# segments-ai/latent-diffusion-segmentation

Measured on AMD Instinct MI355X. Metric: denoising-steps/sec, higher is better.
Workload: dtype bf16; 1 GPU; 512x512 COCO-shaped latents (64x64x4), batch 8 per GPU, DDIM, self-conditioned 12-ch UNet without cross-attention (BASELINE configs[1]); batch_per_gpu=8, global_batch=8, latent=64, parallelism=dp1, ranks=1, backend=none, visible_devices=1

## Files before the change

### include/ldmseg_hip_ops.h

```cpp
#ifndef LDMSEG_HIP_OPS_H_
#define LDMSEG_HIP_OPS_H_
#include <stdint.h>
#ifdef __cplusplus
extern "C" {
#endif

int ldmseg_op_conv2d(const float* x, const float* x2, const float* w, const float* bias, int B, int Ci, int Ci2, int H,
                     int W, int Co, int k, int stride, int up, int dtype, float* out, void* stream);
int ldmseg_op_linear(const float* x, const float* w, const float* bias, const float* resid, const float* rowbias,
                     int rows_per_image, int M, int K, int N, int geglu, int silu, int splits, int dtype, float* out,
                     void* stream);
int ldmseg_op_chained_ff_out(const float* g, const float* h, const float* x, const float* w2, const float* b2, const float* wp,
                             const float* bp, int M, int C, int rows_per_image, int dtype, float* out, void* stream);
int ldmseg_op_groupnorm(const float* x, const float* x2, const float* gamma, const float* beta, int B, int C, int C2,
                        int HW, float eps, int silu, int dtype, float* out, void* stream);
int ldmseg_op_layernorm(const float* x, const float* gamma, const float* beta, int M, int C, float eps, int silu,
                        int dtype, float* out, void* stream);
int ldmseg_op_attention(const float* qkv, int B, int N, int C, int heads, int dtype, float* out, void* stream);
int ldmseg_op_attention_causal(const float* qkv, int B, int N, int C, int heads, int dtype, float* out, void* stream);
int ldmseg_op_attention_cross(const float* q, const float* kv, int B, int N, int S, int C, int heads, int dtype, float* out,
                              void* stream);
int ldmseg_op_attention_fp8(const float* qkv, int B, int N, int C, int heads, float* out, int time_iters, float* us_per_launch,
                            void* stream);
int ldmseg_op_convt2(const float* x, const float* w, const float* bias, int B, int Ci, int H, int W, int Co, int dtype,
                     float* out, void* stream);
int ldmseg_op_bilinear2x(const float* x, int B, int C, int H, int W, int dtype, float* out, void* stream);

int ldmseg_op_panoptic_from_decoder(const float* x4, int B, int C, int H4, int W4, int dtype, int in_h, int in_w,
                                    const int32_t* crop_boxes, const int32_t* out_sizes, const int64_t* out_offsets,
                                    int threshold_output, int threshold_mode, float mask_th, int count_th, double overlap_th,
                                    int64_t ignore_label, int32_t* labels, int32_t* panoptic, uint8_t* keep, int32_t* counts,
                                    int32_t* mask_counts, float* volume, void* stream);

int ldmseg_op_semseg_from_decoder(const float* x4, int B, int C, int H4, int W4, int dtype, int out_h, int out_w, float mask_th,
                                  int64_t ignore_label, const int64_t* targets, int64_t ignore_index, int num_classes,
                                  int64_t* preds, int64_t* counts, float* volume, void* stream);

int ldmseg_op_transformer_in(const float* x, const float* wp, const float* bp, const float* gamma, const float* beta, const float* wq,
                             const float* wk, const float* wv, int M, int C, float eps, int dtype, int mode, float* h_out, float* qkv_out,
                             int time_iters, float* us_per_call, void* stream);
int ldmseg_op_gn_transformer_in(const float* x, const float* gn_gamma, const float* gn_beta, float gn_eps, int images, int gn_mode,
                                const float* wp, const float* bp, const float* gamma, const float* beta, const float* wq,
                                const float* wk, const float* wv, int M, int C, float eps, int dtype, int mode, float* h_out,
                                float* qkv_out, int time_iters, float* us_per_call, void* stream);

int ldmseg_op_igemm(const float* x, const float* x2, const float* w, const float* bias, const float* resid,
                    const float* rowbias, int B, int Ci, int Ci2, int H, int W, int Co, int k, int stride, int up, int geglu,
                    int silu, int splits, int dtype, float* out, void* stream);
int ldmseg_op_conv3x3_plus_1x1(const float* h, const float* w2, const float* b2, const float* xs, const float* xs2, const float* ws,
                               const float* bs, int B, int C, int Cs, int Cs2, int H, int W, int Co, int splits, int dtype, float* out,
                               int iters, float* us_per_launch, void* stream);
int ldmseg_op_conv_groupnorm(const float* x, const float* w, const float* bias, const float* rowbias, const float* gamma,
                             const float* beta, int B, int Ci, int H, int W, int Co, float eps, int silu, int splits, int dtype,
                             float* out, void* stream);
int ldmseg_op_ln_linear(const float* x, const float* gamma, const float* beta, const float* w, const float* bias, int M, int K,
                        int N, float eps, int geglu, int dtype, float* out, void* stream);
int ldmseg_op_ln_linear_silu(const float* x, const float* gamma, const float* beta, const float* w, const float* bias, int M,
                             int K, int N, float eps, int dtype, float* out, void* stream);
int ldmseg_op_clip_patch_rows(const float* img, int B, int H, int W, int S, int P, const float* mean, const float* std,
                              int resample, int dtype, float* out, void* stream);
int ldmseg_op_clip_text_tokens(const int64_t* ids, const float* tok, const float* pos, int R, int T, int C, int vocab, int dtype,
                               float* out, void* stream);
int ldmseg_op_clip_text_final_ln(const float* x, const float* gamma, const float* beta, int M, int C, float eps, int dtype,
                                 float* out, void* stream);
int ldmseg_op_transformer_ff(const float* h, const float* x, const float* gamma, const float* beta, const float* w1, const float* b1,
                             const float* w2, const float* b2, const float* wp, const float* bp, int M, int C, float eps, int dtype,
                             int mode, float* out, int time_iters, float* us_per_call, void* stream);
int ldmseg_op_conv_out_tail(const float* x, const float* w, const float* bias, int B, int H, int W, float* eps_out, int ddim, int last,
                            const float* coef4, int pred_type, int clip, float clip_range, float* latents, float* cond,
                            const float* rgb, const uint8_t* known, const float* z0, const float* noise, float sa, float sb,
                            float* xin_out, void* stream);
int ldmseg_bench_igemm(const float* x, const float* x2, const float* w, const float* bias, const float* resid,
                       const float* rowbias, int B, int Ci, int Ci2, int H, int W, int Co, int k, int stride, int up, int geglu,
                       int silu, int splits, int dtype, int iters, float* us_per_launch, void* stream);
int ldmseg_bench_groupnorm(const float* gamma, const float* beta, int B, int C, int C2, int HW, int silu, int dtype, int iters,
                           float* us_per_launch, void* stream);
int ldmseg_bench_attention(const float* qkv, int B, int N, int C, int heads, int dtype, int iters, float* us_per_launch,
                           void* stream);
int ldmseg_igemm_last_kernel(char* buf, int n);
int ldmseg_op_igemm_plan(const int* desc, int dtype, int cus, char* buf, int n);
int ldmseg_op_groupnorm_plan(int B, int C, int C2, int HW, int groups, int dtype, int cus, int region_ok, char* buf, int n);
int ldmseg_op_conv_groupnorm_plan(int B, int Co, int HW, int dtype, char* buf, int n);
int ldmseg_op_attention_plan(int kind, int B, int N, int S, int C, int heads, int dtype, char* buf, int n);
int ldmseg_igemm_log(int enable);
int ldmseg_igemm_log_read(char* buf, int n);

int ldmseg_op_fastdiv(const int* n, int count, int d, int* q, void* stream);

#ifdef __cplusplus
}
#endif
#endif
```

### latent-diffusion-segmentation_amd/csrc/engine.hip

```cpp
#include <hip/hip_runtime.h>

#include <algorithm>
#include <array>
#include <cmath>
#include <cstdio>
#include <cstring>
#include <string>
#include <unordered_map>
#include <vector>

#include "../../include/ldmseg_hip.h"
#include "attn_plan.h"
#include "kernels.h"

using namespace ldmseg;

namespace {

thread_local std::string g_err;
int g_plan_epoch = 0;
int g_gnfold_mode = 1;
int g_ffp_mode = 1;
int fail(int code, const std::string& msg) {
  g_err = msg;
// ... 2148 lines not shown
  float* e1 = sinus + (size_t)h->temb_cap * 320;
  float* emb = e1 + (size_t)h->temb_cap * kTimeDim;
  float* table = emb + (size_t)h->temb_cap * kTimeDim;
  HIP_TRY(hipMemcpyAsync(ts, timesteps, (size_t)n_steps * sizeof(int64_t), hipMemcpyHostToDevice, s));
  for (int i0 = 0; i0 < n_steps; i0 += 64) {
    const int r = n_steps - i0 < 64 ? n_steps - i0 : 64;
    TRY(launch_time_embed(ts + i0, r, 0, r, sinus + (size_t)i0 * 320, s));
    TRY(launch_small_linear(sinus + (size_t)i0 * 320, h->te1_w, h->te1_b, e1 + (size_t)i0 * kTimeDim, r, 320, kTimeDim, 0, 1, s));
    TRY(launch_small_linear(e1 + (size_t)i0 * kTimeDim, h->te2_w, h->te2_b, emb + (size_t)i0 * kTimeDim, r, kTimeDim, kTimeDim, 0, 0, s));
    TRY(launch_small_linear(emb + (size_t)i0 * kTimeDim, h->tproj_w, h->tproj_b, table + (size_t)i0 * h->temb_total, r, kTimeDim,
                            h->temb_total, 1, 0, s));
  }
  *rows = table;
  return 0;
}

static int loop_reserve(ldmseg_unet* h, size_t n) {
  if (h->loop_elems >= n) return 0;
  HIP_TRY(hipDeviceSynchronize());
  if (h->cond) (void)hipFree(h->cond);
  if (h->eps) (void)hipFree(h->eps);
  h->cond = h->eps = nullptr;
  h->loop_elems = 0;
  HIP_TRY(hipMalloc((void**)&h->cond, n * sizeof(float)));
  HIP_TRY(hipMalloc((void**)&h->eps, n * sizeof(float)));
  h->loop_elems = n;
  return 0;
}

int ldmseg_unet_set_attention_fp8(ldmseg_unet* h, int min_tokens) {
  g_err.clear();
  if (!h || min_tokens < 0) return fail(LDMSEG_E_ARG, "bad argument");
  if (min_tokens > 0 && h->dt != DT_BF16) return fail(LDMSEG_E_ARG, "the fp8 attention path belongs to the bf16 perf mode");
  h->attn_fp8_min_tokens = min_tokens;
  h->plan_valid = false;
  return 0;
}

int ldmseg_unet_reserve(ldmseg_unet* h, int B, int L) {
  g_err.clear();
  if (!h) return fail(LDMSEG_E_ARG, "null argument");
  if (B < 1 || L < 8 || L % 8 != 0) return fail(LDMSEG_E_SHAPE, "L must be a positive multiple of 8, B >= 1");
  DeviceGuard dg(h->cfg.device);
  const int ci = h->cfg.in_channels;
  const PlanKey key{B, L, h->ctx_S, h->ctx_dim};
  TRY(plan_workspace(*h, &key, [&](bool dry, size_t scratch_base) {
    return unet_forward_impl(h, nullptr, ci, nullptr, 0, nullptr, 0, nullptr, 1, 0, B, L, nullptr, nullptr, dry, scratch_base);
  }));
  TRY(loop_reserve(h, (size_t)B * 4 * L * L));
  TRY(temb_reserve(h, 64));
  TRY(igemm_warm());
  return 0;
}

static int gn_backoff_update(ldmseg_unet* h) {
  if (h->gn_sync) {
    if (!h->gn_diag_host) {
      HIP_TRY(hipHostMalloc((void**)&h->gn_diag_host, sizeof(unsigned long long)));
      *h->gn_diag_host = 0;
    }
    const unsigned long long cur = *(volatile unsigned long long*)h->gn_diag_host;
    if (cur >= h->gn_diag_seen + 256) h->gn_backoff_calls = 8;
    else if (h->gn_backoff_calls > 0) --h->gn_backoff_calls;
    h->gn_diag_seen = cur;
  }
  return 0;
}

int ldmseg_sample_loop(ldmseg_unet* h, const ldmseg_sample_cfg* cfg, float* latents, const float* rgb_latents, int B, int L,
                       float* all_latents, void* stream) {
  g_err.clear();
  if (!h || !cfg || !latents || !rgb_latents || !cfg->timesteps || !cfg->coef) return fail(LDMSEG_E_ARG, "null argument");
  if (h->cfg.cross_attention) return fail(LDMSEG_E_ARG, "cross-attention handle: sample with ldmseg_sample_loop_guided");
  if (cfg->n_steps < 1) return fail(LDMSEG_E_ARG, "n_steps must be >= 1");
  if (B < 1 || L < 8 || L % 8 != 0) return fail(LDMSEG_E_SHAPE, "L must be a positive multiple of 8, B >= 1");
  if (cfg->prediction_type < 0 || cfg->prediction_type > 2) return fail(LDMSEG_E_ARG, "unknown prediction_type");
  for (int i = 0; i < cfg->n_steps; ++i)
    if (cfg->timesteps[i] < 0) return fail(LDMSEG_E_ARG, "negative timestep");
  DeviceGuard dg(h->cfg.device);
  hipStream_t s = (hipStream_t)stream;
  const size_t n = (size_t)B * 4 * L * L;
  const bool selfc = cfg->self_condition != 0;
  if ((h->cfg.in_channels == 12) != selfc) return fail(LDMSEG_E_ARG, "self_condition needs the 12-channel conv_in (and vice versa)");
  TRY(loop_reserve(h, n));
  const bool inpaint = cfg->known_dev != nullptr;
  if (inpaint && (!cfg->z0_dev || !cfg->noise_dev || !cfg->paste_coef)) return fail(LDMSEG_E_ARG, "inpainting needs z0, noise and paste_coef");
  if (selfc) HIP_TRY(hipMemsetAsync(h->cond, 0, n * sizeof(float), s));
  const float* temb_rows = nullptr;
  TRY(loop_time_embeddings(h, cfg->timesteps, cfg->n_steps, s, &temb_rows));
  TRY(gn_backoff_update(h));
  struct Clear { ldmseg_unet* u; ~Clear() { u->temb_override = nullptr; u->tail_req = nullptr; u->tail_done = false; u->xin_ready = false; u->xin_ptr = nullptr; } } clear{h};
  for (int i = 0; i < cfg->n_steps; ++i) {
    h->temb_override = temb_rows + (size_t)i * h->temb_total;
    const float* c = cfg->coef + 4 * i;
    DdimCoef dc{c[0], c[1], c[2], c[3], cfg->prediction_type, cfg->clip_sample, cfg->clip_sample_range, 0};
    const bool last = (i == cfg->n_steps - 1);
    StepTail st;
    st.ddim = 1; st.last = last ? 1 : 0; st.c = dc; st.latents = latents; st.cond = selfc ? h->cond : nullptr; st.rgb = rgb_latents;
    if (inpaint) { st.known = cfg->known_dev; st.z0 = cfg->z0_dev; st.noise = cfg->noise_dev; st.sa = cfg->paste_coef[2 * i]; st.sb = cfg->paste_coef[2 * i + 1]; }
    h->tail_req = &st;
    h->tail_done = false;
    TRY(unet_forward_checked(h, latents, 4, rgb_latents, 4, selfc ? h->cond : nullptr, selfc ? 4 : 0, nullptr, 1,
                             cfg->timesteps[i], B, L, h->eps, s));
    h->tail_req = nullptr;
    if (!h->tail_done) {
      if (!last) {
        TRY(launch_ddim_step(h->eps, latents, latents, selfc ? h->cond : nullptr, n, dc, s));
      } else {
        TRY(launch_ddim_step(h->eps, latents, nullptr, latents, n, dc, s));
      }
      if (inpaint)
        TRY(launch_inpaint_paste(latents, cfg->z0_dev, cfg->noise_dev, cfg->known_dev, cfg->paste_coef[2 * i],
                                 cfg->paste_coef[2 * i + 1], B, 4, L * L, s));
    }
    if (all_latents)
      HIP_TRY(hipMemcpyAsync(all_latents + (size_t)i * n, latents, n * sizeof(float), hipMemcpyDeviceToDevice, s));
  }
  if (h->gn_sync && h->gn_diag_host)
    HIP_TRY(hipMemcpyAsync(h->gn_diag_host, gn_sync_diag_ptr(h->gn_sync), sizeof(unsigned long long), hipMemcpyDeviceToHost, s));
  return 0;
}

int ldmseg_sample_loop_guided(ldmseg_unet* h, const ldmseg_sample_cfg* cfg, float* latents, const float* rgb_latents, int B, int L,
                              const float* ctx, int S, int ctx_dim, int multiplier, float guidance_scale, float* all_latents,
                              void* stream) {
  g_err.clear();
  if (!h || !cfg || !latents || !rgb_latents || !cfg->timesteps || !cfg->coef) return fail(LDMSEG_E_ARG, "null argument");
  if (cfg->n_steps < 1) return fail(LDMSEG_E_ARG, "n_steps must be >= 1");
  if (B < 1 || L < 8 || L % 8 != 0) return fail(LDMSEG_E_SHAPE, "L must be a positive multiple of 8, B >= 1");
  if (cfg->prediction_type < 0 || cfg->prediction_type > 2) return fail(LDMSEG_E_ARG, "unknown prediction_type");
  if (multiplier != 1 && multiplier != 2) return fail(LDMSEG_E_ARG, "multiplier must be 1 or 2");
  for (int i = 0; i < cfg->n_steps; ++i)
    if (cfg->timesteps[i] < 0) return fail(LDMSEG_E_ARG, "negative timestep");
  const bool selfc = cfg->self_condition != 0;
  if (selfc && multiplier == 2) return fail(LDMSEG_E_ARG, "self_condition with classifier-free guidance (multiplier 2) is not defined");
  if ((h->cfg.in_channels == 12) != selfc) return fail(LDMSEG_E_ARG, "self_condition needs the 12-channel conv_in (and vice versa)");
  if (cfg->known_dev || cfg->z0_dev || cfg->noise_dev || cfg->paste_coef) return fail(LDMSEG_E_ARG, "inpainting is not combined with guidance");
  TRY(set_ctx(h, ctx, S, ctx_dim));
  CtxClear cc{h};
  DeviceGuard dg(h->cfg.device);
  hipStream_t s = (hipStream_t)stream;
  const size_t n = (size_t)B * 4 * L * L;
  const int BB = multiplier * B;
  TRY(loop_reserve(h, (size_t)multiplier * n));
  float *lat2 = nullptr, *rgb2 = nullptr;
  if (multiplier == 2) {
    if (h->guide_elems < 4 * n) {
      HIP_TRY(hipDeviceSynchronize());
      if (h->guide_buf) (void)hipFree(h->guide_buf);
      h->guide_buf = nullptr; h->guide_elems = 0;
      HIP_TRY(hipMalloc((void**)&h->guide_buf, 4 * n * sizeof(float)));
      h->guide_elems = 4 * n;
    }
    lat2 = h->guide_buf;
    rgb2 = h->guide_buf + 2 * n;
    for (int k = 0; k < 2; ++k) {
      HIP_TRY(hipMemcpyAsync(lat2 + k * n, latents, n * sizeof(float), hipMemcpyDeviceToDevice, s));
      HIP_TRY(hipMemcpyAsync(rgb2 + k * n, rgb_latents, n * sizeof(float), hipMemcpyDeviceToDevice, s));
    }
  }
  if (selfc) HIP_TRY(hipMemsetAsync(h->cond, 0, n * sizeof(float), s));
  const float* temb_rows = nullptr;
  TRY(loop_time_embeddings(h, cfg->timesteps, cfg->n_steps, s, &temb_rows));
  TRY(gn_backoff_update(h));
  struct Clear { ldmseg_unet* u; ~Clear() { u->temb_override = nullptr; u->xin_ready = false; u->xin_ptr = nullptr; } } clear{h};
  for (int i = 0; i < cfg->n_steps; ++i) {
    h->temb_override = temb_rows + (size_t)i * h->temb_total;
    const float* c = cfg->coef + 4 * i;
    DdimCoef dc{c[0], c[1], c[2], c[3], cfg->prediction_type, cfg->clip_sample, cfg->clip_sample_range, 0};
    const bool last = (i == cfg->n_steps - 1);
    TRY(unet_forward_checked(h, multiplier == 2 ? lat2 : latents, 4, multiplier == 2 ? rgb2 : rgb_latents, 4,
                             selfc ? h->cond : nullptr, selfc ? 4 : 0, nullptr, 1, cfg->timesteps[i], BB, L, h->eps, s));
    h->ctx_kv_ready = true;
    TRY(launch_guided_step(h->eps, latents, selfc ? h->cond : nullptr, lat2, n, multiplier, guidance_scale, dc, last ? 1 : 0, s));
    if (all_latents)
      HIP_TRY(hipMemcpyAsync(all_latents + (size_t)i * n, latents, n * sizeof(float), hipMemcpyDeviceToDevice, s));
  }
  if (h->gn_sync && h->gn_diag_host)
    HIP_TRY(hipMemcpyAsync(h->gn_diag_host, gn_sync_diag_ptr(h->gn_sync), sizeof(unsigned long long), hipMemcpyDeviceToHost, s));
  return 0;
}

int ldmseg_unet_cf_fallbacks(ldmseg_unet* h, int64_t* count) {
  g_err.clear();
  if (!h || !count) return fail(LDMSEG_E_ARG, "null argument");
  DeviceGuard dg(h->cfg.device);
  unsigned long long n = 0;
  if (h->cf_sync) {
    HIP_TRY(hipDeviceSynchronize());
    HIP_TRY(hipMemcpy(&n, (const unsigned long long*)h->cf_sync + igemm_cf_bytes() / 8 - 1, sizeof n, hipMemcpyDeviceToHost));
  }
  *count = (int64_t)n;
  return 0;
}

int ldmseg_unet_gn_backoff(ldmseg_unet* h, int32_t* calls_left) {
  g_err.clear();
  if (!h || !calls_left) return fail(LDMSEG_E_ARG, "null argument");
  *calls_left = h->gn_backoff_calls;
  return 0;
}

int ldmseg_unet_gn_fallbacks(ldmseg_unet* h, int64_t* count) {
  g_err.clear();
  if (!h || !count) return fail(LDMSEG_E_ARG, "null argument");
  DeviceGuard dg(h->cfg.device);
  const long long n = h->gn_sync ? gn_coop_fallbacks(h->gn_sync) : 0;
  if (n < 0) return fail(LDMSEG_E_HIP, "reading the GroupNorm fallback counter failed");
  *count = n;
  return 0;
}

int ldmseg_bit_encode(const int64_t* ids, int B, int n_bits, int HW, int64_t ignore_label, float fill_value, float mul,
                      float add, float* bits, uint8_t* ignore_mask, void* stream) {
  g_err.clear();
  if (!ids || !bits || n_bits < 1 || n_bits > 31) return fail(LDMSEG_E_ARG, "bad bit_encode argument");
  TRY(launch_bit_encode(ids, bits, ignore_mask, B, n_bits, HW, ignore_label, fill_value, mul, add, (hipStream_t)stream));
  return 0;
}
int ldmseg_bit_decode(const float* x, int B, int n_bits, int HW, int64_t* ids, void* stream) {
  g_err.clear();
  if (!x || !ids || n_bits < 1 || n_bits > 24) return fail(LDMSEG_E_ARG, "bad bit_decode argument");
  TRY(launch_bit_decode(x, ids, B, n_bits, HW, (hipStream_t)stream));
  return 0;
}

int ldmseg_panoptic_postprocess(const float* logits, int B, int C, int H, int W, int threshold_output, int threshold_mode,
                                float mask_th, int count_th, double overlap_th, int64_t ignore_label, int32_t* labels,
                                int32_t* panoptic, uint8_t* keep, int32_t* counts, int32_t* mask_counts, void* stream) {
  g_err.clear();
  if (!logits || !labels || !panoptic || !keep || !counts || !mask_counts || B < 1 || C < 1 || C > 256 || H < 1 || W < 1 ||
      (threshold_mode != 0 && threshold_mode != 1))
    return fail(LDMSEG_E_ARG, "bad panoptic_postprocess argument");
  TRY(launch_panoptic_postprocess(logits, B, C, H * W, threshold_output, threshold_mode, mask_th, count_th, overlap_th,
                                  ignore_label, labels, panoptic, keep, counts, mask_counts, (hipStream_t)stream));
  return 0;
}

int ldmseg_profile_enable(int enable) {
  g_prof.on = enable != 0;
  return 0;
}
int ldmseg_profile_reset(void) {
  for (auto& f : g_prof.fam) {
    for (auto& e : f.ev) { g_prof.pool.push_back(e.first); g_prof.pool.push_back(e.second); }
    f.ev.clear();
    f.label.clear();
    f.lflops.clear();
    f.launches = 0;
    f.flops = f.bytes = 0;
  }
  return 0;
}
int ldmseg_profile_read(int family, int64_t* launches, double* total_ms, double* flops, double* bytes) {
  g_err.clear();
  if (family < 0 || family > 4) return fail(LDMSEG_E_ARG, "family must be 0..4");
  ProfFamily& f = g_prof.fam[family];
  double ms = 0;
  for (auto& e : f.ev) {
    HIP_TRY(hipEventSynchronize(e.second));
    float t = 0;
    HIP_TRY(hipEventElapsedTime(&t, e.first, e.second));
    ms += t;
  }
  if (launches) *launches = f.launches;
  if (total_ms) *total_ms = ms;
  if (flops) *flops = f.flops;
  if (bytes) *bytes = f.bytes;
  return 0;
}

int ldmseg_debug_set(int key, int value) {
  if (key == 2) { attention_set_qf1(value); return 0; }
  if (key == 1) { igemm_set_dbg(value); ++g_plan_epoch; return 0; }
  if (key == 5) { igemm_force_cfg(value); ++g_plan_epoch; return 0; }
  if (key == 8) { groupnorm_set_variant(value); ++g_plan_epoch; return 0; }
  if (key == 9) { igemm_set_cm_mode(value); ++g_plan_epoch; return 0; }
  if (key == 10) { groupnorm_set_coop(value, groupnorm_knob(11)); return 0; }
  if (key == 11) { groupnorm_set_coop(groupnorm_knob(10), value); return 0; }
  if (key == 12) { mlp_fused_set_mode(value); ++g_plan_epoch; return 0; }
  if (key == 13) { mlp_fused_set_dbg(value); return 0; }
  if (key == 14) { step_tail_set_mode(value); ++g_plan_epoch; return 0; }
  if (key == 16) { proj_qkv_set_mode(value); ++g_plan_epoch; return 0; }
  if (key == 15) { attention_mx_set_mode(value); ++g_plan_epoch; return 0; }
  if (key == 23) { igemm_set_cf_mode(value); ++g_plan_epoch; return 0; }
  if (key == 24) { igemm_set_table_override(value); ++g_plan_epoch; return 0; }
  if (key == 19) { igemm_set_xt_mode(value); ++g_plan_epoch; return 0; }
  if (key == 20) { g_ffp_mode = value ? 1 : 0; ++g_plan_epoch; return 0; }
  if (key == 22) { g_gnfold_mode = value < 0 ? 0 : value; ++g_plan_epoch; return 0; }
  if (key == 21) { igemm_set_up4_mode(value); ++g_plan_epoch; return 0; }
  if (key == 6 || key == 7) { ops_bench_knob(key, value); return 0; }
  static unsigned long long ts_ptr = 0;
  if (key == 3) { ts_ptr = (ts_ptr & 0xffffffff00000000ull) | (unsigned)value; igemm_set_tsbuf((void*)(uintptr_t)ts_ptr); return 0; }
  if (key == 4) { ts_ptr = (ts_ptr & 0xffffffffull) | ((unsigned long long)(unsigned)value << 32); igemm_set_tsbuf((void*)(uintptr_t)ts_ptr); return 0; }
  return fail(LDMSEG_E_ARG, "unknown debug key");
}

int ldmseg_debug_get(int key) {
  if (key == 1) return igemm_get_dbg();
  if (key == -1) return igemm_default_dbg();
  if (key == 8 || key == 11) return groupnorm_knob(key);
  if (key == 9) return igemm_get_cm_mode();
  if (key == 12) return mlp_fused_get_mode();
  if (key == 14) return step_tail_get_mode();
  if (key == 16) return proj_qkv_get_mode();
  if (key == 15) return attention_mx_get_mode();
  if (key == 23) return igemm_get_cf_mode();
  if (key == 19) return igemm_get_xt_mode();
  if (key == 20) return g_ffp_mode;
  if (key == 22) return g_gnfold_mode;
  if (key == 21) return igemm_get_up4_mode();
  if (key == 10) { const long long n = gn_coop_fallbacks(nullptr); return n > 0x7fffffffll ? 0x7fffffff : (int)n; }
  return 0;
}

int ldmseg_igemm_last_kernel(char* buf, int n) {
  if (!buf || n < 1) return LDMSEG_E_ARG;
  std::snprintf(buf, (size_t)n, "%s", igemm_dispatch_line(igemm_last_dispatch()).c_str());
  return 0;
}
int ldmseg_igemm_log(int enable) { igemm_log_enable(enable); return 0; }
int ldmseg_igemm_log_read(char* buf, int n) {
  if (!buf || n < 1) return LDMSEG_E_ARG;
  const std::string s = igemm_log_read();
  if ((int)s.size() + 1 > n) return LDMSEG_E_ARG;
  std::memcpy(buf, s.c_str(), s.size() + 1);
  return 0;
}

int ldmseg_profile_dump(const char* path) {
  g_err.clear();
  FILE* fp = std::fopen(path, "w");
  if (!fp) return fail(LDMSEG_E_ARG, "cannot open profile dump file");
  std::fprintf(fp, "family,label,ms,flops\n");
  for (int fi = 0; fi < 5; ++fi) {
    ProfFamily& f = g_prof.fam[fi];
    for (size_t i = 0; i < f.ev.size(); ++i) {
      (void)hipEventSynchronize(f.ev[i].second);
      float t = 0;
      (void)hipEventElapsedTime(&t, f.ev[i].first, f.ev[i].second);
      std::fprintf(fp, "%d,%s,%.6f,%.0f\n", fi, i < f.label.size() ? f.label[i].c_str() : "", t,
                   i < f.lflops.size() ? f.lflops[i] : 0.0);
    }
  }
  std::fclose(fp);
  return 0;
}

}
```

### latent-diffusion-segmentation_amd/csrc/kernels.h

```cpp
#pragma once
#include <hip/hip_runtime.h>
#include <stdint.h>

#include <string>
#include <vector>

#include "igemm_types.h"

namespace ldmseg {

struct FastDiv {
  unsigned mul = 0;
  int shift = 0;
  int d = 1;
};
inline FastDiv fastdiv_make(int d) {
  FastDiv f;
  f.d = d < 1 ? 1 : d;
  if (f.d == 1) return f;
  int s = 0;
  while ((1ll << s) < f.d) ++s;
  const unsigned long long num = 1ull << (31 + s);
  f.mul = (unsigned)((num + (unsigned long long)f.d - 1) / (unsigned long long)f.d);
  f.shift = s - 1;
  return f;
}

struct IgemmParams {
  const void* src0 = nullptr;
  const void* src1 = nullptr;
  int C0 = 0, C1 = 0;
  const void* src2 = nullptr;
  const void* src3 = nullptr;
  int C2 = 0, C3 = 0;
  int B = 0, Hi = 0, Wi = 0, Ho = 0, Wo = 0;
  int taps = 1;
  int pad = -1;
  int stride = 1;
  int up = 0;
  int up4 = 0;
  int cm = 0;
  int M = 0;
  int N = 0;
  int n_valid = 0;
  const void* W = nullptr;
  const float* bias = nullptr;
  const float* rowbias = nullptr;
  int rb_stride = 0;
  const float* rowstats = nullptr;
  const float* c1 = nullptr;
  const void* resid = nullptr;
  int ldr = 0;
  void* out = nullptr;
  int ldo = 0;
  int epi = EPI_STORE;
  int silu = 0;
  int cout = 0;
  int splits = 1;
  float* partial = nullptr;
  int no_finish = 0;
  unsigned long long* cf_ctr = nullptr;
  int cf = 0;
  unsigned cf_bytes = 0;
  int cf_poll_ticks = 20000;
  int cf_diag = 0;
  const void* zeros = nullptr;
  FastDiv fd_hwo, fd_wo, fd_nt, fd_ntiles, fd_nsplit, fd_tpt, fd_mphase;
  int x3 = 0;
  int w_dynamic = 0;
  int dbg = 0;
  unsigned long long* ts = nullptr;
};

int launch_igemm(const IgemmParams& p, int dtype, hipStream_t s);
size_t igemm_partial_bytes(const IgemmParams& p);
int igemm_warm();
int num_cus();
int igemm_plan_splits(const IgemmParams& p, int dtype);
size_t igemm_cf_bytes();
void igemm_set_cf_mode(int mode);
int igemm_get_cf_mode();
void igemm_set_table_override(int v);
void attention_set_qf1(int v);
void igemm_set_tsbuf(void* dev_buf);
void igemm_set_dbg(int flags);
void ops_bench_knob(int key, int value);
void igemm_set_cm_mode(int mode);
int igemm_get_cm_mode();
bool igemm_conv_cm(int hw, int ctot, int n, int k, int stride, int up, int dtype);
bool igemm_up4_ok(int B, int H, int W, int C, int N, int dtype);
void igemm_set_up4_mode(int on);
int igemm_get_up4_mode();
int launch_pack_up4(const float* w, void* out, int Co, int Ci, int Npad, int Cipad, int dtype, hipStream_t s);
bool igemm_xt_ok(const IgemmParams& p, int dtype);
void igemm_set_xt_mode(int on);
int igemm_get_xt_mode();
int launch_chain_weights(const float* wp, const float* w2, const float* b2, const float* bp, float* wcat, float* bcat, int C, hipStream_t s);
int launch_vec_add(const float* a, const float* b, float* out, int n, hipStream_t s);
int launch_split_planes(void* w, size_t nfloats, hipStream_t s);
int launch_concat_rows(const void* a, int K1, const void* b, int K2, void* out, int N, int dtype, hipStream_t s);
void igemm_force_cfg(int cfg);
int igemm_get_dbg();
int igemm_default_dbg();
IgemmDispatch igemm_last_dispatch();
int igemm_plan(const IgemmLaunchDesc& desc, int dtype, int cus, IgemmDispatch* d);
std::string igemm_dispatch_name(const IgemmDispatch& d);
std::string igemm_dispatch_line(const IgemmDispatch& d);
void igemm_log_enable(int level);
int igemm_log_level();
void igemm_log_note(const char* name);
std::string igemm_log_read();
std::string launch_name(const char* fmt, ...);
template <typename T>
constexpr const char* dtype_tag() { return sizeof(T) == 2 ? "bf16" : "f32"; }
#define LDMSEG_LAUNCH_AT(LEVEL, NAME, ...)                                                                  \
  do {                                                                                                      \
    if (::ldmseg::igemm_log_level() >= (LEVEL)) ::ldmseg::igemm_log_note(std::string(NAME).c_str());        \
    hipLaunchKernelGGL(__VA_ARGS__);                                                                        \
  } while (0)
#define LDMSEG_LAUNCH_GEMM(NAME, ...) LDMSEG_LAUNCH_AT(1, NAME, __VA_ARGS__)
#define LDMSEG_LAUNCH(NAME, ...) LDMSEG_LAUNCH_AT(2, NAME, __VA_ARGS__)
int igemm_pick_bn(int n_real, int epi);

struct GNParams {
  const void* src0 = nullptr; const void* src1 = nullptr;
  int C0 = 0, C1 = 0, B = 0, HW = 0, groups = 32;
  const float* gamma = nullptr; const float* beta = nullptr;
  float eps = 1e-5f; int silu = 0;
  void* out = nullptr;
  float* partial = nullptr;
  int nchunk = 0;
  int cpg = 0, vx = 0, ty = 0, per = 0;
  FastDiv fd_cpg, fd_vx, fd_aux;
  double inv_n = 0.0;
  void* sync_region = nullptr;
  unsigned long long* sync = nullptr;
  unsigned long long* sync_ctr = nullptr;
  unsigned long long* sync_diag = nullptr;
  int splits = 1;
  int coop_mode = 0;
  int poll_ticks = 10000;
  int poll_us = -1;
};
size_t gn_sync_bytes();
int gn_sync_init(void* region, hipStream_t s);
int gn_warm();
void groupnorm_set_coop(int mode, int poll_us);
long long gn_coop_fallbacks(const void* region);
const void* gn_sync_diag_ptr(const void* region);
int gn_nchunk(int B, int HW);
int launch_groupnorm(const GNParams& p, int dtype, hipStream_t s);
int launch_groupnorm_stats(const GNParams& p, int dtype, hipStream_t s);
bool finish_groupnorm_ok(int B, int HW, int C, int dtype);
int launch_finish_groupnorm(const IgemmParams& ip, const GNParams& g, int dtype, hipStream_t s);
void groupnorm_set_variant(int v);
int groupnorm_knob(int key);
struct GnDesc;
struct GnPlan;
int groupnorm_plan(const GnDesc& q, int cus, bool region_ok, GnPlan* pl);
int finish_groupnorm_plan(int B, int HW, int C, int dtype, GnPlan* pl);

int launch_layernorm(const void* x, void* y, const float* gamma, const float* beta, int M, int C,
                     float eps, int silu, int dtype, hipStream_t s);

int launch_attention(const void* qkv, void* out, int B, int N, int C, int heads, int dtype, hipStream_t s);
int launch_attention_causal(const void* qkv, void* out, int B, int N, int C, int heads, int dtype, hipStream_t s);
struct AttnKnobs;
struct AttnPlan;
AttnKnobs attention_knobs();
int launch_attn_v1_plan(const AttnPlan& p, const void* qkv, void* out, hipStream_t s);
int launch_attn3_plan(const AttnPlan& p, const void* qkv, void* out, hipStream_t s);
int launch_attn4_plan(const AttnPlan& p, const void* qkv, void* out, hipStream_t s);
int launch_attn_fp8_plan(const AttnPlan& p, const void* qkv, void* kv8, void* out, hipStream_t s);
int launch_attn_mx_plan(const AttnPlan& p, const void* qkv, void* kv8, void* out, hipStream_t s);
int launch_attn_cross_plan(const AttnPlan& p, const void* q, const void* kv, void* out, hipStream_t s);

int launch_attention_cross(const void* q, const void* kv, void* out, int B, int N, int S, int C, int heads, int dtype, hipStream_t s);
int launch_rows_to_dtype(const float* x, void* y, size_t n, int dtype, hipStream_t s);

bool mlp_fused_ok(int C, int dtype);
bool mlp_fused_proj();
void mlp_fused_set_mode(int m);
int mlp_fused_get_mode();
size_t mlp_fused_stream_bytes(int C);
int launch_pack_mlp_stream(const void* w1, const void* w2, const void* wp, void* out, int C, hipStream_t s);
bool proj_qkv_fused_ok(int C, int M, int dtype);
void proj_qkv_set_mode(int m);
int proj_qkv_get_mode();
size_t proj_qkv_stream_bytes(int C);
int launch_pack_proj_qkv_stream(const void* wp, const void* wqkv, void* out, int C, hipStream_t s);
struct GnFold {
  const float* partial = nullptr;
  const float* gamma = nullptr;
  const float* beta = nullptr;
  int nchunk = 0, HW = 0;
  float eps = 1e-6f;
};
bool proj_qkv_gn_fold_ok(int HW);
int proj_qkv_gn_chunks(int B, int HW);
int launch_proj_qkv_fused(const void* x, void* h, void* qkv, const void* stream, const float* bias4, const void* zeros, int M, int C, float eps,
                          const GnFold* gn, hipStream_t s);
int launch_mlp_fused(const void* h, void* out, const void* x2, const void* stream, const float* bias1, const float* bias2,
                     const float* bias3, const void* zeros, int M, int C, float eps, int proj, int rows_per_image, hipStream_t s);
void mlp_fused_set_dbg(int flags);
const void* igemm_zero_page();

int launch_rowstats(const void* x, float* stats, int M, int C, float eps, int dtype, hipStream_t s);
int launch_repack_rows_scaled(const float* w, void* out, const int* src_row_dev, int Npad, int K, const float* colscale,
                              int dtype, hipStream_t s);
int launch_rowsum(const void* W, const float* add, float* out, int N, int K, int dtype, hipStream_t s);

std::vector<int> geglu_row_map(int nout);
int launch_padded_bias(const float* src, int n, float* dst, int Npad, hipStream_t s);
struct LnFold {
  int parts = 1;
  const float* w[3] = {};
  const float* bias[3] = {};
  int Nper = 0, K = 0;
  int Npad = 0;
  const float* gamma = nullptr;
  const float* beta = nullptr;
  const std::vector<int>* row_map = nullptr;
  float scale = 0.f;
  int dtype = DT_BF16;
};
size_t ln_fold_scratch_bytes(const LnFold& f);
int launch_ln_fold(const LnFold& f, void* scratch, void* W, float* c1, float* bias, hipStream_t s);

int launch_clip_patch_rows(const float* img, void* rows, int B, int H, int W, int S, int P, int Kpad, const float* mean,
                           const float* std, int resample, int dtype, hipStream_t s);
int launch_clip_tokens(const void* patch, const float* cls, const float* pos, const float* gamma, const float* beta, void* h,
                       int B, int T, int C, float eps, int dtype, hipStream_t s);
int launch_clip_pooled_ln(const void* h, const float* gamma, const float* beta, float* out, int B, int T, int C, float eps,
                          int dtype, hipStream_t s);
int launch_clip_rows_to_f32(const void* x, float* y, size_t n, int dtype, hipStream_t s);

int launch_clip_text_tokens(const int64_t* ids, const float* tok, const float* pos, void* h, int R, int T, int C, int vocab,
                            int dtype, hipStream_t s);
int launch_clip_text_final_ln(const void* h, const float* gamma, const float* beta, float* out, int M, int C, float eps, int dtype,
                              hipStream_t s);

size_t attention_fp8_scratch_bytes(int B, int N, int C, int heads);
int launch_attention_fp8(const void* qkv, void* kv8_scratch, void* out, int B, int N, int C, int heads, hipStream_t s);
void attention_mx_set_mode(int m);
int attention_mx_get_mode();

int launch_pack_nchw(const float* x, void* y, int B, int C, int HW, int Cpad, float mul, float add,
                     int dtype, hipStream_t s);
int launch_pack_concat3(const float* a, int Ca, const float* b, int Cb, const float* c, int Cc,
                        void* y, int B, int HW, int Cpad, int dtype, hipStream_t s);

int launch_time_embed(const int64_t* t_dev, int t_count, int64_t t_host, int B, float* sinus ,
                      hipStream_t s);
int launch_small_linear(const float* x, const float* W, const float* bias, float* y, int B, int K, int N,
                        int silu_in, int silu_out, hipStream_t s);

int launch_bilinear2x_nchw(const void* x, float* y, int B, int H, int W, int C, int dtype, hipStream_t s);

int launch_bilinear2x_argmax(const void* x, int64_t* ids, float* prob, int B, int H, int W, int C, float mask_th,
                             int64_t ignore_label, int dtype, hipStream_t s);

int launch_repack_conv(const float* w, void* out, int Co, int Ci, int KH, int KW, int Npad, int Cipad,
                       int dtype, hipStream_t s, int cm_tile = 0);
int launch_repack_rows(const float* w, void* out, const int* src_row_dev, int Npad, int K, int dtype, hipStream_t s);
int launch_repack_convt2(const float* w, void* out, int Ci, int Co, int dtype, hipStream_t s);

struct DdimCoef { float sqrt_a_t, sqrt_b_t, sqrt_a_prev, sqrt_b_prev; int pred_type; int clip; float clip_range; int use_clipped; };
int launch_ddim_step(const float* eps, const float* x, float* prev, float* x0, size_t n, DdimCoef c, hipStream_t s);
int launch_guided_step(const float* eps, float* latents, float* cond, float* lat2, size_t n, int mult, float g, DdimCoef c,
                       int last, hipStream_t s);
struct StepTail {
  const void* x = nullptr;
  const void* w = nullptr;
  const float* bias = nullptr;
  const void* zeros = nullptr;
  int B = 0, H = 0, W = 0;
  float* eps_out = nullptr;
  int ddim = 0, last = 0;
  DdimCoef c{};
  float* latents = nullptr;
  float* cond = nullptr;
  const float* rgb = nullptr;
  void* xin_next = nullptr;
  const uint8_t* known = nullptr; const float* z0 = nullptr; const float* noise = nullptr;
  float sa = 0.f, sb = 0.f;
};
bool conv_out_tail_ok(int C, int H, int W, int dtype);
bool step_tail_fused();
void step_tail_set_mode(int m);
int step_tail_get_mode();
int launch_conv_out_tail(const StepTail& t, hipStream_t s);
int launch_inpaint_paste(float* cur, const float* z0, const float* noise, const uint8_t* known, float sa, float sb,
                         int B, int C, int HW, hipStream_t s);
int launch_add_noise(const float* x0, const float* noise, const int64_t* t_dev, const float* ac_dev, int n_train, float scale,
                     float* out, int B, size_t per, int remove, hipStream_t s);
int launch_softmax_rows(const float* s, void* p, int rows, int n, float scale, int dtype, hipStream_t st);
int launch_axpby(const float* x, float a, float b, float* y, size_t n, hipStream_t s);
int launch_panoptic_postprocess(const float* logits, int B, int C, int HW, int threshold_output, int threshold_mode,
                                float mask_th, int count_th, double overlap_th, int64_t ignore_label, int32_t* labels,
                                int32_t* panoptic, uint8_t* keep, int32_t* counts, int32_t* mask_counts, hipStream_t s);
int launch_panoptic_from_decoder(const void* x4, int B, int H4, int W4, int C, int dtype, int in_h, int in_w,
                                 const int32_t* boxes_host, const int32_t* sizes_host, const int64_t* offsets_host,
                                 int threshold_output, int threshold_mode, float mask_th, int count_th, double overlap_th,
                                 int64_t ignore_label, int32_t* labels, int32_t* panoptic, uint8_t* keep, int32_t* counts,
                                 int32_t* mask_counts, hipStream_t s, float* volume = nullptr,
                                 int mask_rule = 0);
int launch_semseg_meter(const int64_t* pred, const int64_t* gt, size_t n, int K, int64_t ignore_index, int64_t* counts, hipStream_t s);
int launch_semseg_from_decoder(const void* x4, int B, int H4, int W4, int C, int dtype, int oh, int ow, float mask_th,
                               int64_t ignore_label, const int64_t* targets, int64_t ignore_index, int K, int64_t* preds,
                               int64_t* counts, hipStream_t s, float* volume = nullptr);
int launch_pq_match(const int32_t* pred, const void* gt, int gt_format, int B, const int32_t* sizes_host, const int64_t* pred_offsets_host,
                    const int64_t* gt_offsets_host, const uint8_t* keep, int P, const int32_t* gt_counts_host, int Gpad,
                    const int32_t* slot_ids, const uint8_t* slot_crowd, const int64_t* slot_area, const int32_t* slot_meta,
                    int32_t* inter, int32_t* stats, double* match_iou, hipStream_t s);
int launch_bit_encode(const int64_t* ids, float* out, uint8_t* ignore, int B, int n, int HW, int64_t ignore_label,
                      float fill, float mul, float add, hipStream_t s);
int launch_bit_decode(const float* x, int64_t* out, int B, int n, int HW, hipStream_t s);
int launch_posterior_sample(const float* moments, const float* noise, float* out, int B, int HW, hipStream_t s);

}
```

### latent-diffusion-segmentation_amd/csrc/ops_api.hip

```cpp
#include <hip/hip_runtime.h>

#include <string>
#include <cstdio>
#include <cstdlib>
#include <cstring>
#include <vector>

#include "../../include/ldmseg_hip.h"
#include "common.h"
#include "attn_plan.h"
#include "gn_plan.h"
#include "kernels.h"

using namespace ldmseg;

static unsigned long long* op_cf_region() {
  static unsigned long long* r[64] = {};
  int dev = 0;
  if (hipGetDevice(&dev) != hipSuccess || dev < 0 || dev >= 64) return nullptr;
  if (!r[dev]) {
    void* q = nullptr;
    if (hipMalloc(&q, igemm_cf_bytes()) != hipSuccess) return nullptr;
    (void)hipMemset(q, 0, igemm_cf_bytes());
    r[dev] = (unsigned long long*)q;
// ... 373 lines not shown
  hipStream_t s = (hipStream_t)stream;
  if (M < 1 || C < 1) return -2;
  Temp t;
  void* xp = t.get((size_t)M * C * es(dtype));
  to_dev_dtype(x, xp, (size_t)M * C, dtype, s);
  return launch_clip_text_final_ln(xp, gamma, beta, out, M, C, eps, dtype, s);
}

int ldmseg_op_attention_cross(const float* q, const float* kv, int B, int N, int S, int C, int heads, int dtype, float* out,
                              void* stream) {
  hipStream_t s = (hipStream_t)stream;
  if (B < 1 || N < 1 || S < 1 || heads < 1 || C % heads) return -2;
  Temp t;
  void* qp = t.get((size_t)B * N * C * es(dtype));
  to_dev_dtype(q, qp, (size_t)B * N * C, dtype, s);
  void* kp = t.get((size_t)B * S * 2 * C * es(dtype));
  to_dev_dtype(kv, kp, (size_t)B * S * 2 * C, dtype, s);
  void* op = t.get((size_t)B * N * C * es(dtype));
  const int r = launch_attention_cross(qp, kp, op, B, N, S, C, heads, dtype, s);
  if (r) return r;
  from_dev_dtype(op, out, (size_t)B * N * C, dtype, s);
  return 0;
}

int ldmseg_op_convt2(const float* x, const float* w, const float* bias, int B, int Ci, int H, int W, int Co, int dtype,
                     float* out, void* stream) {
  hipStream_t s = (hipStream_t)stream;
  Temp t;
  if (Ci % bke(dtype) || Co % 4) return -2;
  void* xp = t.get((size_t)B * H * W * Ci * es(dtype));
  if (launch_pack_nchw(x, xp, B, Ci, H * W, Ci, 1.f, 0.f, dtype, s)) return -3;
  const int N = 4 * Co;
  const int bn = igemm_pick_bn(N, EPI_STORE);
  const int Np = rupi(N, bn);
  void* wp = t.get((size_t)Np * Ci * es(dtype));
  (void)hipMemsetAsync(wp, 0, (size_t)Np * Ci * es(dtype), s);
  if (launch_repack_convt2(w, wp, Ci, Co, dtype, s)) return -3;
  float* bp = (float*)t.get(Np * sizeof(float));
  (void)hipMemsetAsync(bp, 0, Np * sizeof(float), s);
  if (bias) for (int q = 0; q < 4; ++q) (void)hipMemcpyAsync(bp + q * Co, bias, Co * sizeof(float), hipMemcpyDeviceToDevice, s);
  void* op = t.get((size_t)B * 4 * H * W * Co * es(dtype));
  IgemmParams p;
  p.src0 = xp; p.C0 = Ci; p.B = B; p.Hi = p.Ho = H; p.Wi = p.Wo = W; p.M = B * H * W; p.N = Np; p.n_valid = N;
  p.W = wp; p.bias = bp; p.out = op; p.ldo = Co; p.epi = EPI_CONVT2; p.cout = Co;
  const int r = launch_igemm(p, dtype, s);
  if (r) return r;
  return unpack_nhwc(op, out, B, Co, 4 * H * W, Co, dtype, s);
}

int ldmseg_op_bilinear2x(const float* x, int B, int C, int H, int W, int dtype, float* out, void* stream) {
  hipStream_t s = (hipStream_t)stream;
  Temp t;
  void* xp = t.get((size_t)B * H * W * C * es(dtype));
  if (launch_pack_nchw(x, xp, B, C, H * W, C, 1.f, 0.f, dtype, s)) return -3;
  return launch_bilinear2x_nchw(xp, out, B, H, W, C, dtype, s);
}

static int g_bench_rot = 1, g_bench_ln = 0;
static int op_igemm_impl(const float* x, const float* x2, const float* w, const float* bias, const float* resid,
                         const float* rowbias, int B, int Ci, int Ci2, int H, int W, int Co, int k, int stride, int up, int geglu,
                         int silu, int splits, int dtype, float* out, void* stream, int time_iters, float* us_per_launch) {
  hipStream_t s = (hipStream_t)stream;
  Temp t;
  const int x3 = dtype == 2 ? 1 : (dtype == 3 ? 2 : 0);
  if (x3) dtype = DT_F32;
  const int a = bke(dtype);
  const int c0 = rupi(Ci, a), c1 = Ci2 ? rupi(Ci2, a) : 0;
  if (Ci2 && (Ci % a)) return -2;
  if (geglu && (k != 1 || Ci2 || (Co % 32))) return -2;
  void* xp = t.get((size_t)B * H * W * c0 * es(dtype));
  void* x2p = Ci2 ? t.get((size_t)B * H * W * c1 * es(dtype)) : nullptr;
  if (launch_pack_nchw(x, xp, B, Ci, H * W, c0, 1.f, 0.f, dtype, s)) return -3;
  if (Ci2 && launch_pack_nchw(x2, x2p, B, Ci2, H * W, c1, 1.f, 0.f, dtype, s)) return -3;
  const int epi = geglu ? EPI_GEGLU : EPI_STORE;
  const int bn = igemm_pick_bn(Co, epi);
  const int Np = rupi(Co, bn);
  const int ct = c0 + c1;
  const int cout = geglu ? Co / 2 : Co;
  const bool cm = !geglu && igemm_conv_cm(H * W, c0 + c1, Np, k, stride, up, dtype) && (Ci % a) == 0 && (!Ci2 || (Ci2 % a) == 0);
  void* wp = t.get((size_t)Np * k * k * ct * es(dtype));
  float* bp = padded_bias(t, geglu ? nullptr : bias, Co, Np, s);
  if (geglu) {
    std::vector<int> map = geglu_row_map(cout);
    map.resize(Np, -1);
    const int* dmap = upload_map(t, map, s);
    if (launch_repack_rows(w, wp, dmap, Np, ct, dtype, s)) return -3;
    if (bias && launch_repack_rows(bias, bp, dmap, Np, 1, DT_F32, s)) return -3;
  } else if (!Ci2) {
    if (launch_repack_conv(w, wp, Co, Ci, k, k, Np, c0, dtype, s, cm ? a : 0)) return -3;
  } else {
    void* w_cat = t.get((size_t)Co * ct * k * k * sizeof(float));
    (void)hipMemsetAsync(w_cat, 0, (size_t)Co * ct * k * k * sizeof(float), s);
    (void)hipMemcpy2DAsync(w_cat, (size_t)ct * k * k * sizeof(float), w, (size_t)(Ci + Ci2) * k * k * sizeof(float),
                           (size_t)(Ci + Ci2) * k * k * sizeof(float), Co, hipMemcpyDeviceToDevice, s);
    if (launch_repack_conv((const float*)w_cat, wp, Co, ct, k, k, Np, ct, dtype, s, cm ? a : 0)) return -3;
  }
  const int Hl = up ? 2 * H : H, Wl = up ? 2 * W : W;
  const int Ho = (k == 3 && stride == 2) ? (Hl - 1) / 2 + 1 : Hl, Wo = (k == 3 && stride == 2) ? (Wl - 1) / 2 + 1 : Wl;
  void* rp = nullptr;
  if (resid) {
    rp = t.get((size_t)B * Ho * Wo * cout * es(dtype));
    if (launch_pack_nchw(resid, rp, B, cout, Ho * Wo, cout, 1.f, 0.f, dtype, s)) return -3;
  }
  void* op = t.get((size_t)B * Ho * Wo * cout * es(dtype));
  IgemmParams p;
  p.src0 = xp; p.C0 = c0; p.src1 = x2p; p.C1 = c1;
  p.B = B; p.Hi = H; p.Wi = W; p.Ho = Ho; p.Wo = Wo; p.taps = k * k; p.stride = stride; p.up = up; p.cm = cm ? 1 : 0;
  p.M = B * Ho * Wo; p.N = Np; p.n_valid = cout; p.W = wp; p.bias = bp;
  p.rowbias = rowbias; p.rb_stride = Co;
  p.resid = rp; p.ldr = cout; p.out = op; p.ldo = cout; p.epi = epi; p.silu = silu;
  p.x3 = x3;
  if (x3 == 2 && launch_split_planes(wp, (size_t)Np * k * k * ct, s)) return -3;
  if (up && k == 3 && stride == 1 && !Ci2 && !geglu && !resid && !rowbias && !silu && igemm_up4_ok(B, H, W, c0, Np, dtype) && Ci == c0) {
    void* w4 = t.get((size_t)16 * Np * c0 * es(dtype));
    if (launch_pack_up4(w, w4, Co, Ci, Np, c0, dtype, s)) return -3;
    p.W = w4; p.taps = 4; p.up = 0; p.up4 = 1; p.Ho = H; p.Wo = W; p.M = 4 * B * H * W; p.cm = 0;
  }
  p.cf_ctr = op_cf_region();
  int sp = splits > 0 ? splits : igemm_plan_splits(p, dtype);
  if (sp > 1) { p.splits = sp; p.partial = (float*)t.get((size_t)sp * p.M * Np * sizeof(float)); }
  if (time_iters > 0 && g_bench_ln && sp <= 1 && !rowbias) {
    float* st = (float*)t.get((size_t)p.M * 2 * sizeof(float));
    float* c1z = (float*)t.get(Np * sizeof(float));
    (void)hipMemsetAsync(c1z, 0, Np * sizeof(float), s);
    std::vector<float> h((size_t)p.M * 2);
    for (int m = 0; m < p.M; ++m) { h[2 * m] = 0.f; h[2 * m + 1] = 1.f; }
    (void)hipMemcpy(st, h.data(), h.size() * sizeof(float), hipMemcpyHostToDevice);
    p.rowstats = st; p.c1 = c1z;
  }
  const int r = launch_igemm(p, dtype, s);
  if (r) return r;
  if (time_iters > 0 && us_per_launch) {
    const size_t wbytes = p.up4 ? (size_t)16 * Np * c0 * es(dtype) : (size_t)Np * k * k * ct * es(dtype);
    const void* wsrc = p.W;
    int rot = g_bench_rot < 1 ? 1 : g_bench_rot;
    std::vector<const void*> wc(1, wsrc);
    for (int i = 1; i < rot; ++i) {
      void* c = t.get(wbytes);
      if (!c) break;
      (void)hipMemcpyAsync(c, wsrc, wbytes, hipMemcpyDeviceToDevice, s);
      wc.push_back(c);
    }
    rot = (int)wc.size();
    *us_per_launch = time_launches(s, 3, time_iters, [&](int i) { p.W = wc[i % rot]; (void)launch_igemm(p, dtype, s); });
  }
  if (!out) return 0;
  return unpack_nhwc(op, out, B, cout, Ho * Wo, cout, dtype, s);
}

int ldmseg_op_conv3x3_plus_1x1(const float* h, const float* w2, const float* b2, const float* xs, const float* xs2, const float* ws,
                               const float* bs, int B, int C, int Cs, int Cs2, int H, int W, int Co, int splits, int dtype, float* out,
                               int iters, float* us_per_launch, void* stream) {
  hipStream_t s = (hipStream_t)stream;
  Temp t;
  if (dtype != DT_BF16 || C % 64 || Cs % 64 || Cs2 % 64 || !h || !w2 || !xs || !ws) return -2;
  const int HW = H * W, cs = Cs + Cs2;
  void* hp = t.get((size_t)B * HW * C * 2);
  void* xp = t.get((size_t)B * HW * Cs * 2);
  void* x2p = Cs2 ? t.get((size_t)B * HW * Cs2 * 2) : nullptr;
  if (launch_pack_nchw(h, hp, B, C, HW, C, 1.f, 0.f, dtype, s)) return -3;
  if (launch_pack_nchw(xs, xp, B, Cs, HW, Cs, 1.f, 0.f, dtype, s)) return -3;
  if (Cs2 && launch_pack_nchw(xs2, x2p, B, Cs2, HW, Cs2, 1.f, 0.f, dtype, s)) return -3;
  const int Np = rupi(Co, igemm_pick_bn(Co, EPI_STORE));
  void* w2p = t.get((size_t)Np * 9 * C * 2);
  void* wsp = t.get((size_t)Np * cs * 2);
  void* wx = t.get((size_t)Np * (9 * C + cs) * 2);
  if (launch_repack_conv(w2, w2p, Co, C, 3, 3, Np, C, dtype, s)) return -3;
  if (launch_repack_conv(ws, wsp, Co, cs, 1, 1, Np, cs, dtype, s)) return -3;
  if (launch_concat_rows(w2p, 9 * C, wsp, cs, wx, Np, dtype, s)) return -3;
  float* b2p = padded_bias(t, b2, Co, Np, s);
  float* bsp = padded_bias(t, bs, Co, Np, s);
  float* bx = (float*)t.get(Np * sizeof(float));
  if (launch_vec_add(b2p, bsp, bx, Np, s)) return -3;
  void* op = t.get((size_t)B * HW * Co * 2);
  IgemmParams p;
  p.src0 = hp; p.C0 = C; p.src2 = xp; p.C2 = Cs; p.src3 = x2p; p.C3 = Cs2;
  p.B = B; p.Hi = p.Ho = H; p.Wi = p.Wo = W; p.taps = 9; p.stride = 1;
  p.M = B * HW; p.N = Np; p.n_valid = Co; p.W = wx; p.bias = bx; p.out = op; p.ldo = Co; p.epi = EPI_STORE;
  if (!igemm_xt_ok(p, dtype)) return -4;
  p.cf_ctr = op_cf_region();
  const int sp = splits > 0 ? splits : igemm_plan_splits(p, dtype);
  if (sp > 1) { p.splits = sp; p.partial = (float*)t.get((size_t)sp * p.M * Np * sizeof(float)); }
  const int r = launch_igemm(p, dtype, s);
  if (r) return r;
  if (iters > 0 && us_per_launch) *us_per_launch = time_launches(s, 0, iters, [&](int) { (void)launch_igemm(p, dtype, s); });
  if (!out) return 0;
  return unpack_nhwc(op, out, B, Co, HW, Co, dtype, s);
}

int ldmseg_op_igemm_plan(const int* desc, int dtype, int cus, char* buf, int n) {
  if (!desc || !buf || n < 1 || cus < 1 || dtype < 0 || dtype > 3) return -2;
  IgemmLaunchDesc q;
  static_assert(sizeof q == 17 * sizeof(int), "ldmseg_op_igemm_plan takes the fields of IgemmLaunchDesc in order");
  std::memcpy(&q, desc, sizeof q);
  if (dtype >= 2) { q.x3 = dtype - 1; dtype = DT_F32; }
  IgemmDispatch d;
  if (const int r = igemm_plan(q, dtype, cus, &d)) return r;
  std::snprintf(buf, (size_t)n, "%s", igemm_dispatch_line(d).c_str());
  return 0;
}

int ldmseg_op_fastdiv(const int* n, int count, int d, int* q, void* stream) {
  if (!n || !q || count < 0 || d < 1) return -2;
  const FastDiv f = fastdiv_make(d);
  hipLaunchKernelGGL(fastdiv_probe_kernel, dim3((count + 255) / 256), dim3(256), 0, (hipStream_t)stream, n, count, f, q);
  return hipGetLastError() == hipSuccess ? 0 : -3;
}
}
namespace ldmseg {
void ops_bench_knob(int key, int value) {
  if (key == 6) g_bench_rot = value;
  if (key == 7) g_bench_ln = value;
}
}
extern "C" {
int ldmseg_op_igemm(const float* x, const float* x2, const float* w, const float* bias, const float* resid,
                    const float* rowbias, int B, int Ci, int Ci2, int H, int W, int Co, int k, int stride, int up, int geglu,
                    int silu, int splits, int dtype, float* out, void* stream) {
  return op_igemm_impl(x, x2, w, bias, resid, rowbias, B, Ci, Ci2, H, W, Co, k, stride, up, geglu, silu, splits, dtype, out,
                       stream, 0, nullptr);
}
int ldmseg_bench_igemm(const float* x, const float* x2, const float* w, const float* bias, const float* resid,
                       const float* rowbias, int B, int Ci, int Ci2, int H, int W, int Co, int k, int stride, int up, int geglu,
                       int silu, int splits, int dtype, int iters, float* us_per_launch, void* stream) {
  return op_igemm_impl(x, x2, w, bias, resid, rowbias, B, Ci, Ci2, H, W, Co, k, stride, up, geglu, silu, splits, dtype, nullptr,
                       stream, iters, us_per_launch);
}
int ldmseg_bench_attention(const float* qkv, int B, int N, int C, int heads, int dtype, int iters, float* us_per_launch,
                           void* stream) {
  hipStream_t s = (hipStream_t)stream;
  Temp t;
  void* qp = t.get((size_t)B * N * 3 * C * es(dtype));
  to_dev_dtype(qkv, qp, (size_t)B * N * 3 * C, dtype, s);
  void* op = t.get((size_t)B * N * C * es(dtype));
  int err = 0;
  *us_per_launch = time_launches(s, 3, iters, [&](int) { if (const int r = launch_attention(qp, op, B, N, C, heads, dtype, s)) err = err ? err : r; });
  return err;
}

}
namespace {
int op_ln_linear_impl(const float* x, const float* gamma, const float* beta, const float* w, const float* bias, int M, int K,
                      int N, float eps, int geglu, int silu, int dtype, float* out, void* stream) {
  hipStream_t s = (hipStream_t)stream;
  Temp t;
  const int x3 = dtype == 2 ? 1 : (dtype == 3 ? 2 : 0);
  if (x3) dtype = DT_F32;
  if (K % bke(dtype)) return -2;
  void* xp = t.get((size_t)M * K * es(dtype));
  to_dev_dtype(x, xp, (size_t)M * K, dtype, s);
  const int epi = geglu ? EPI_GEGLU : EPI_STORE;
  const int bn = (!geglu && N % 160 != 0) ? 160 : igemm_pick_bn(N, epi);
  const int Np = rupi(N, bn);
  const int nout = geglu ? N / 2 : N;
  std::vector<int> map;
  if (geglu) { map = geglu_row_map(nout); map.resize(Np, -1); }
  LnFold f;
  f.w[0] = w; f.bias[0] = bias; f.Nper = N; f.K = K; f.Npad = Np; f.gamma = gamma; f.beta = beta; f.dtype = dtype;
  if (geglu) f.row_map = &map;
  void* wp = t.get((size_t)Np * K * es(dtype));
  float* c1 = (float*)t.get(Np * sizeof(float));
  float* c2 = (float*)t.get(Np * sizeof(float));
  if (launch_ln_fold(f, t.get(ln_fold_scratch_bytes(f)), wp, c1, c2, s)) return -3;
  float* stats = (float*)t.get((size_t)M * 2 * sizeof(float));
  if (launch_rowstats(xp, stats, M, K, eps, dtype, s)) return -3;
  void* op = t.get((size_t)M * nout * es(dtype));
  IgemmParams p;
  p.src0 = xp; p.C0 = K; p.B = 1; p.Hi = p.Ho = M; p.Wi = p.Wo = 1;
  p.M = M; p.N = Np; p.n_valid = nout; p.W = wp; p.bias = c2; p.rowstats = stats; p.c1 = c1;
  p.out = op; p.ldo = nout; p.epi = epi; p.silu = silu;
  p.x3 = x3;
  if (x3 == 2 && launch_split_planes(wp, (size_t)Np * K, s)) return -3;
  const int sp = igemm_plan_splits(p, dtype);
  if (sp > 1) { p.splits = sp; p.partial = (float*)t.get((size_t)sp * M * Np * sizeof(float)); }
  const int r = launch_igemm(p, dtype, s);
  if (r) return r;
  from_dev_dtype(op, out, (size_t)M * nout, dtype, s);
  return 0;
}
}
extern "C" {
int ldmseg_op_ln_linear(const float* x, const float* gamma, const float* beta, const float* w, const float* bias, int M, int K,
                        int N, float eps, int geglu, int dtype, float* out, void* stream) {
  return op_ln_linear_impl(x, gamma, beta, w, bias, M, K, N, eps, geglu, 0, dtype, out, stream);
}
int ldmseg_op_ln_linear_silu(const float* x, const float* gamma, const float* beta, const float* w, const float* bias, int M,
                             int K, int N, float eps, int dtype, float* out, void* stream) {
  return op_ln_linear_impl(x, gamma, beta, w, bias, M, K, N, eps, 0, 1, dtype, out, stream);
}
int ldmseg_op_clip_patch_rows(const float* img, int B, int H, int W, int S, int P, const float* mean, const float* std,
                              int resample, int dtype, float* out, void* stream) {
  hipStream_t s = (hipStream_t)stream;
  if (B < 1 || P < 1 || S < P || S % P) return -2;
  Temp t;
  const int Kpad = rupi(3 * P * P, 64), G = S / P;
  const size_t n = (size_t)B * G * G * Kpad;
  void* rows = t.get(n * es(dtype));
  const int r = launch_clip_patch_rows(img, rows, B, H, W, S, P, Kpad, mean, std, resample, dtype, s);
  if (r) return r;
  from_dev_dtype(rows, out, n, dtype, s);
  return 0;
}

int ldmseg_op_transformer_ff(const float* h, const float* x, const float* gamma, const float* beta, const float* w1, const float* b1,
                             const float* w2, const float* b2, const float* wp, const float* bp, int M, int C, float eps, int dtype,
                             int mode, float* out, int time_iters, float* us_per_call, void* stream) {
  hipStream_t s = (hipStream_t)stream;
  Temp t;
  const int rows_per_image = (M % 4096 == 0) ? 4096 : 0;
  if (C % bke(dtype) || (mode != 0 && (dtype != DT_BF16 || !mlp_fused_stream_bytes(C)))) return -2;
  const int N1 = 8 * C;
  void* hp = t.get((size_t)M * C * es(dtype));
  void* h0 = t.get((size_t)M * C * es(dtype));
  void* xp = t.get((size_t)M * C * es(dtype));
  void* op = t.get((size_t)M * C * es(dtype));
  to_dev_dtype(h, h0, (size_t)M * C, dtype, s);
  to_dev_dtype(x, xp, (size_t)M * C, dtype, s);
  const std::vector<int> map = geglu_row_map(4 * C);
  LnFold f;
  f.w[0] = w1; f.bias[0] = b1; f.Nper = N1; f.K = C; f.Npad = N1; f.gamma = gamma; f.beta = beta; f.row_map = &map; f.dtype = dtype;
  void* w1p = t.get((size_t)N1 * C * es(dtype));
  float* c1 = (float*)t.get(N1 * sizeof(float));
  float* c2 = (float*)t.get(N1 * sizeof(float));
  if (launch_ln_fold(f, t.get(ln_fold_scratch_bytes(f)), w1p, c1, c2, s)) return -3;
  void* w2p = t.get((size_t)C * 4 * C * es(dtype));
  void* wpp = t.get((size_t)C * C * es(dtype));
  to_dev_dtype(w2, w2p, (size_t)C * 4 * C, dtype, s);
  to_dev_dtype(wp, wpp, (size_t)C * C, dtype, s);
  float* b2d = (float*)t.get(C * sizeof(float));
  float* bpd = (float*)t.get(C * sizeof(float));
  (void)hipMemcpyAsync(b2d, b2, C * sizeof(float), hipMemcpyDeviceToDevice, s);
  (void)hipMemcpyAsync(bpd, bp, C * sizeof(float), hipMemcpyDeviceToDevice, s);
  void* stream_w = nullptr;
  if (mode != 0) {
    stream_w = t.get(mlp_fused_stream_bytes(C));
    if (launch_pack_mlp_stream(w1p, w2p, wpp, stream_w, C, s)) return -3;
  }
  float* stats = (float*)t.get((size_t)M * 2 * sizeof(float));
  void* ff = t.get((size_t)M * 4 * C * es(dtype));
  if (igemm_warm()) return -3;
  auto gemm = [&](const void* src, int K, const void* W, int N, int nvalid, const float* bias, const void* resid, void* o, int epi,
                  const float* rs, const float* cc1) -> int {
    IgemmParams p;
    p.src0 = src; p.C0 = K; p.B = 1; p.Hi = p.Ho = M; p.Wi = p.Wo = 1;
    p.M = M; p.N = N; p.n_valid = nvalid; p.W = W; p.bias = bias; p.rowstats = rs; p.c1 = cc1;
    p.resid = resid; p.ldr = C; p.out = o; p.ldo = nvalid; p.epi = epi;
    const int sp = igemm_plan_splits(p, dtype);
    if (sp > 1) { p.splits = sp; p.partial = (float*)t.get((size_t)sp * M * N * sizeof(float)); }
    return launch_igemm(p, dtype, s);
  };
  auto run = [&]() -> int {
    (void)hipMemcpyAsync(hp, h0, (size_t)M * C * es(dtype), hipMemcpyDeviceToDevice, s);
    if (mode == 0) {
      if (int r = launch_rowstats(hp, stats, M, C, eps, dtype, s)) return r;
      if (int r = gemm(hp, C, w1p, N1, 4 * C, c2, nullptr, ff, EPI_GEGLU, stats, c1)) return r;
      if (int r = gemm(ff, 4 * C, w2p, C, C, b2d, hp, hp, EPI_STORE, nullptr, nullptr)) return r;
      return gemm(hp, C, wpp, C, C, bpd, xp, op, EPI_STORE, nullptr, nullptr);
    }
    const int proj = (mode & 2) ? 1 : 0;
    if (int r = launch_mlp_fused(hp, proj ? op : hp, xp, stream_w, c2, b2d, bpd, igemm_zero_page(), M, C, eps, proj, rows_per_image, s)) return r;
    return proj ? 0 : gemm(hp, C, wpp, C, C, bpd, xp, op, EPI_STORE, nullptr, nullptr);
  };
  if (int r = run()) return r;
  if (time_iters > 0 && us_per_call) *us_per_call = time_launches(s, 2, time_iters, [&](int) { (void)run(); });
  from_dev_dtype(op, out, (size_t)M * C, dtype, s);
  return 0;
}

static int transformer_in_impl(const float* x, const float* gn_gamma, const float* gn_beta, float gn_eps, int gn_images, int gn_mode,
                               const float* wp, const float* bp, const float* gamma, const float* beta, const float* wq,
                               const float* wk, const float* wv, int M, int C, float eps, int dtype, int mode, float* h_out, float* qkv_out,
                               int time_iters, float* us_per_call, void* stream) {
  hipStream_t s = (hipStream_t)stream;
  Temp t;
  if (C % bke(dtype) || (mode != 0 && (dtype != DT_BF16 || !proj_qkv_stream_bytes(C) || M % 128))) return -2;
  GNParams gp;
  GnFold gf;
  void* xn = nullptr;
  if (gn_gamma) {
    if (gn_images < 1 || M % gn_images || C % 32 || (gn_mode == 1 && (mode != 1 || !proj_qkv_gn_fold_ok(M / gn_images)))) return -2;
    xn = t.get((size_t)M * C * es(dtype));
    float* gg = (float*)t.get(C * sizeof(float));
    float* gb = (float*)t.get(C * sizeof(float));
    (void)hipMemcpyAsync(gg, gn_gamma, C * sizeof(float), hipMemcpyDeviceToDevice, s);
    (void)hipMemcpyAsync(gb, gn_beta, C * sizeof(float), hipMemcpyDeviceToDevice, s);
    gp.C0 = C; gp.B = gn_images; gp.HW = M / gn_images; gp.groups = 32; gp.gamma = gg; gp.beta = gb; gp.eps = gn_eps; gp.silu = 0;
    gp.out = xn;
    gp.nchunk = gn_mode == 1 ? proj_qkv_gn_chunks(gp.B, gp.HW) : gn_nchunk(gp.B, gp.HW);
    gp.partial = (float*)t.get((size_t)gp.B * gp.nchunk * 32 * 2 * sizeof(float));
    gf.partial = gp.partial; gf.gamma = gg; gf.beta = gb; gf.nchunk = gp.nchunk; gf.HW = gp.HW; gf.eps = gn_eps;
  }
  void* xp = t.get((size_t)M * C * es(dtype));
  void* hp = t.get((size_t)M * C * es(dtype));
  void* qp = t.get((size_t)M * 3 * C * es(dtype));
  to_dev_dtype(x, xp, (size_t)M * C, dtype, s);
  void* wpp = t.get((size_t)C * C * es(dtype));
  to_dev_dtype(wp, wpp, (size_t)C * C, dtype, s);
  void* wqkv = t.get((size_t)3 * C * C * es(dtype));
  float* bias4 = (float*)t.get((size_t)4 * C * sizeof(float));
  float* c1 = (float*)t.get((size_t)3 * C * sizeof(float));
  (void)hipMemcpyAsync(bias4, bp, C * sizeof(float), hipMemcpyDeviceToDevice, s);
  LnFold f;
  f.parts = 3; f.w[0] = wq; f.w[1] = wk; f.w[2] = wv; f.Nper = C; f.K = C; f.Npad = 3 * C; f.gamma = gamma; f.beta = beta; f.dtype = dtype;
  if (launch_ln_fold(f, t.get(ln_fold_scratch_bytes(f)), wqkv, c1, bias4 + C, s)) return -3;
  void* stream_w = nullptr;
  if (mode != 0) {
    stream_w = t.get(proj_qkv_stream_bytes(C));
    if (launch_pack_proj_qkv_stream(wpp, wqkv, stream_w, C, s)) return -3;
  }
  float* stats = (float*)t.get((size_t)M * 2 * sizeof(float));
  if (igemm_warm()) return -3;
  auto gemm = [&](const void* src, const void* W, int N, const float* bias, void* o, const float* rs, const float* cc1) -> int {
    IgemmParams p;
    p.src0 = src; p.C0 = C; p.B = 1; p.Hi = p.Ho = M; p.Wi = p.Wo = 1;
    p.M = M; p.N = N; p.n_valid = N; p.W = W; p.bias = bias; p.rowstats = rs; p.c1 = cc1;
    p.out = o; p.ldo = N; p.epi = EPI_STORE;
    const int sp = igemm_plan_splits(p, dtype);
    if (sp > 1) { p.splits = sp; p.partial = (float*)t.get((size_t)sp * M * N * sizeof(float)); }
    return launch_igemm(p, dtype, s);
  };
  auto run = [&]() -> int {
    const void* xin = xp;
    if (gn_gamma) {
      gp.src0 = xp;
      if (gn_mode == 1) {
        if (int r = launch_groupnorm_stats(gp, dtype, s)) return r;
        return launch_proj_qkv_fused(xp, hp, qp, stream_w, bias4, igemm_zero_page(), M, C, eps, &gf, s);
      }
      if (int r = launch_groupnorm(gp, dtype, s)) return r;
      xin = xn;
    }
    if (mode == 0) {
      if (int r = gemm(xin, wpp, C, bias4, hp, nullptr, nullptr)) return r;
      if (int r = launch_rowstats(hp, stats, M, C, eps, dtype, s)) return r;
      return gemm(hp, wqkv, 3 * C, bias4 + C, qp, stats, c1);
    }
    return launch_proj_qkv_fused(xin, hp, qp, stream_w, bias4, igemm_zero_page(), M, C, eps, nullptr, s);
  };
  if (int r = run()) return r;
  if (time_iters > 0 && us_per_call) *us_per_call = time_launches(s, 2, time_iters, [&](int) { (void)run(); });
  from_dev_dtype(hp, h_out, (size_t)M * C, dtype, s);
  from_dev_dtype(qp, qkv_out, (size_t)M * 3 * C, dtype, s);
  return 0;
}
int ldmseg_op_transformer_in(const float* x, const float* wp, const float* bp, const float* gamma, const float* beta, const float* wq,
                             const float* wk, const float* wv, int M, int C, float eps, int dtype, int mode, float* h_out, float* qkv_out,
                             int time_iters, float* us_per_call, void* stream) {
  return transformer_in_impl(x, nullptr, nullptr, 0.f, 0, 0, wp, bp, gamma, beta, wq, wk, wv, M, C, eps, dtype, mode, h_out, qkv_out,
                             time_iters, us_per_call, stream);
}
int ldmseg_op_gn_transformer_in(const float* x, const float* gn_gamma, const float* gn_beta, float gn_eps, int images, int gn_mode,
                                const float* wp, const float* bp, const float* gamma, const float* beta, const float* wq,
                                const float* wk, const float* wv, int M, int C, float eps, int dtype, int mode, float* h_out,
                                float* qkv_out, int time_iters, float* us_per_call, void* stream) {
  if (!gn_gamma || !gn_beta) return -2;
  return transformer_in_impl(x, gn_gamma, gn_beta, gn_eps, images, gn_mode, wp, bp, gamma, beta, wq, wk, wv, M, C, eps, dtype, mode, h_out,
                             qkv_out, time_iters, us_per_call, stream);
}

int ldmseg_op_conv_out_tail(const float* x, const float* w, const float* bias, int B, int H, int W, float* eps_out, int ddim, int last,
                            const float* coef4, int pred_type, int clip, float clip_range, float* latents, float* cond,
                            const float* rgb, const uint8_t* known, const float* z0, const float* noise, float sa, float sb,
                            float* xin_out, void* stream) {
  hipStream_t s = (hipStream_t)stream;
  Temp t;
  if (!conv_out_tail_ok(320, H, W, DT_BF16)) return -2;
  void* xp = t.get((size_t)B * H * W * 320 * 2);
  if (launch_pack_nchw(x, xp, B, 320, H * W, 320, 1.f, 0.f, DT_BF16, s)) return -3;
  void* wp = t.get((size_t)32 * 9 * 320 * 2);
  if (launch_repack_conv(w, wp, 4, 320, 3, 3, 32, 320, DT_BF16, s)) return -3;
  float* bp = padded_bias(t, bias, 4, 32, s);
  if (igemm_warm()) return -3;
  StepTail st;
  st.x = xp; st.w = wp; st.bias = bp; st.zeros = igemm_zero_page(); st.B = B; st.H = H; st.W = W; st.eps_out = eps_out;
  void* xin = nullptr;
  if (ddim) {
    if (!coef4 || !latents) return -2;
    st.ddim = 1; st.last = last;
    st.c = DdimCoef{coef4[0], coef4[1], coef4[2], coef4[3], pred_type, clip, clip_range, 0};
    st.latents = latents; st.cond = cond; st.rgb = rgb; st.known = known; st.z0 = z0; st.noise = noise; st.sa = sa; st.sb = sb;
    if (xin_out) { xin = t.get((size_t)B * H * W * 64 * 2); (void)hipMemsetAsync(xin, 0xff, (size_t)B * H * W * 64 * 2, s); st.xin_next = xin; }
  }
  const int r = launch_conv_out_tail(st, s);
  if (r) return r;
  if (xin && !last) from_dev_dtype(xin, xin_out, (size_t)B * H * W * 64, DT_BF16, s);
  return 0;
}

int ldmseg_op_attention_fp8(const float* qkv, int B, int N, int C, int heads, float* out, int time_iters, float* us_per_launch,
                            void* stream) {
  hipStream_t s = (hipStream_t)stream;
  Temp t;
  const size_t kv = attention_fp8_scratch_bytes(B, N, C, heads);
  if (!kv) return -2;
  void* qp = t.get((size_t)B * N * 3 * C * 2);
  to_dev_dtype(qkv, qp, (size_t)B * N * 3 * C, DT_BF16, s);
  void* op = t.get((size_t)B * N * C * 2);
  void* kp = t.get(kv);
  int r = launch_attention_fp8(qp, kp, op, B, N, C, heads, s);
  if (r) return r;
  if (time_iters > 0 && us_per_launch) {
    *us_per_launch = time_launches(s, 2, time_iters, [&](int) { (void)launch_attention_fp8(qp, kp, op, B, N, C, heads, s); });
  }
  if (out) from_dev_dtype(op, out, (size_t)B * N * C, DT_BF16, s);
  return 0;
}

}
```

### latent-diffusion-segmentation_amd/csrc/tfuse.hip

```cpp
#include <hip/hip_runtime.h>

#include "common.h"
#include "kernels.h"

namespace ldmseg {
namespace {

constexpr int kBM = 128;
constexpr int kC = 320;
constexpr int kKT = kC / 64;
constexpr int kHC = 64;
constexpr int kXT = kKT * kBM * 128;
constexpr int kHT = kBM * 128;
constexpr int kRing = 65536;
constexpr int kLds = kXT + kHT + kRing;
constexpr int kW1Tile = 128 * 128;
constexpr int kW2Unit = kC * 128;
constexpr int kChunkBytes = kKT * kW1Tile + kW2Unit;
constexpr int kW2A = 192 * 128, kW2B = 128 * 128;
constexpr int kPUnit = 192 * 128;

__device__ __forceinline__ void glds16(const void* gsrc, unsigned lds_dst) {
  asm volatile(
      "s_mov_b32 m0, %1\n\t"
      "s_nop 0\n\t"
      "global_load_lds_dwordx4 %0, off"
      :
      : "v"(gsrc), "s"(lds_dst)
      : "memory");
}
__device__ __forceinline__ void glds16_sbase(unsigned voff, const void* sbase, unsigned lds_dst) {
  asm volatile(
      "s_mov_b32 m0, %2\n\t"
      "s_nop 3\n\t"
      "global_load_lds_dwordx4 %0, %1"
      :
      : "v"(voff), "s"(sbase), "s"(lds_dst)
      : "memory");
}
__device__ __forceinline__ void glds16x2_sbase(unsigned voff, const void* sbase, unsigned lds_dst) {
  asm volatile(
      "s_mov_b32 m0, %2\n\t"
      "s_nop 3\n\t"
      "global_load_lds_dwordx4 %0, %1\n\t"
      "global_load_lds_dwordx4 %0, %1 offset:1024"
      :
      : "v"(voff), "s"(sbase), "s"(lds_dst)
      : "memory");
}
__device__ __forceinline__ void wait_pieces(int n) {
  switch (n) {
#define TF_W(N) case N: asm volatile("s_waitcnt vmcnt(" #N ")" ::: "memory"); break;
    TF_W(0) TF_W(1) TF_W(2) TF_W(3) TF_W(4) TF_W(5) TF_W(6) TF_W(7) TF_W(8) TF_W(9) TF_W(10) TF_W(11) TF_W(12) TF_W(13)
    TF_W(14) TF_W(15)
#undef TF_W
    default: asm volatile("s_waitcnt vmcnt(16)" ::: "memory"); break;
  }
}

struct MlpFusedParams {
  const bf16_t* x;
  bf16_t* out;
  const bf16_t* x2;
  const unsigned char* stream;
  const float* bias1;
  const float* bias2;
  const float* bias3;
  const void* zeros;
  int M, nchunks;
  float eps;
  int rot_tiles;
  int dbg;
  int ldr_delay;
};
#ifdef LDMSEG_TFUSE_ABLATE
#define TFDBG(p, bit) ((LDMSEG_TFUSE_ABLATE) & (bit))
__device__ unsigned long long g_tf_ts[64];
#define TFSTAMP(slot) if (blockIdx.x == 0 && threadIdx.x == 0) g_tf_ts[slot] = wall_clock64();
#define TFSTAMP_L(slot, cond) if ((cond) && blockIdx.x == 0 && threadIdx.x == 512) g_tf_ts[slot] = wall_clock64();
#else
#define TFDBG(p, bit) 0
#define TFSTAMP(slot)
#define TFSTAMP_L(slot, cond)
#endif

template <bool PROJ>
__global__ __launch_bounds__(768, 3) void mlp_fused_kernel(const MlpFusedParams p) {
  extern __shared__ __attribute__((aligned(16))) unsigned char smem[];
  const int tid = threadIdx.x;
  const int lane = tid & 63;
  const int wave_id = __builtin_amdgcn_readfirstlane(tid >> 6);
  const int m0 = blockIdx.x * kBM;
  const unsigned lds0 = (unsigned)(uintptr_t)((__attribute__((address_space(3))) unsigned char*)smem);
  const int nunits = p.nchunks * 5 + (PROJ ? 2 * kKT : 0);
  const int start = p.rot_tiles > 0 ? (int)(((unsigned)blockIdx.x % (unsigned)p.rot_tiles) * 7u % (unsigned)p.nchunks) : 0;

  if (wave_id >= 8) {
    const int lw = wave_id - 8;
    {
      const int ld_r = lane >> 3, ld_j = (lane & 7) ^ ld_r;
#pragma unroll 4
      for (int i = 0; i < (kKT * kBM / 8) / 4; ++i) {
        const int q = lw + 4 * i;
        const int kt = q >> 4, rg = q & 15;
        const int m = m0 + rg * 8 + ld_r;
        const void* src = m < p.M ? (const void*)((const unsigned char*)p.x + (size_t)m * (kC * 2) + kt * 128 + ld_j * 16) : p.zeros;
        glds16(src, __builtin_amdgcn_readfirstlane(lds0 + kt * (kBM * 128) + rg * 1024));
      }
    }
    __builtin_amdgcn_s_setprio(3);
    const int nchunk_units = p.nchunks * 5;
    const int chunk_pieces = p.nchunks * 30;
    int left = chunk_pieces + (PROJ ? 2 * kKT * 6 : 0);
    int iss = 0;
    const unsigned voff = (unsigned)lane * 16u;
    const unsigned char* src = p.stream + (size_t)start * kChunkBytes + (size_t)lw * 2048;
    int to_wrap = (p.nchunks - start) * 15;
    unsigned dst = (unsigned)lw * 2048u;
    auto issue_n = [&](int n) __attribute__((always_inline)) {
      for (int i = 0; i < n && left > 0; i += 2) {
        if (!TFDBG(p, 1)) {
          const unsigned long long su = (unsigned long long)(uintptr_t)src;
          const unsigned lo = __builtin_amdgcn_readfirstlane((unsigned)su), hi = __builtin_amdgcn_readfirstlane((unsigned)(su >> 32));
          glds16x2_sbase(voff, (const void*)(uintptr_t)(((unsigned long long)hi << 32) | lo),
                         __builtin_amdgcn_readfirstlane(lds0 + (unsigned)(kXT + kHT) + dst));
        }
        src += 8192;
        dst = (dst + 8192u) & (unsigned)(kRing - 1);
        iss += 2;
        left -= 2;
        if (--to_wrap == 0) {
          if (iss < chunk_pieces) { src = p.stream + (size_t)lw * 2048; to_wrap = start * 15; }
          else { src = p.stream + (size_t)p.nchunks * kChunkBytes + (size_t)lw * 2048; to_wrap = 0x7fffffff; }
        }
      }
    };
    issue_n(16);
    wait_pieces(iss);
    __syncthreads();
    int land = 8;
    wait_pieces(iss - land);
    __syncthreads();
    int pos = 0;
    for (int t = 0; t < nunits; ++t) {
      if (PROJ && t == nchunk_units) asm volatile("s_barrier" ::: "memory");
      const int sh_t = (t < nchunk_units) ? ((0x46488 >> (4 * pos)) & 15) : 6;
      if (t + 1 < nunits) {
        const int pn = pos == 4 ? 0 : pos + 1;
        land += (t + 1 < nchunk_units) ? ((0x46488 >> (4 * pn)) & 15) : 6;
        wait_pieces(iss - land);
      }
      asm volatile("s_barrier" ::: "memory");
      if (p.ldr_delay == 1) __builtin_amdgcn_s_sleep(2);
      issue_n(sh_t);
      pos = (pos == 4) ? 0 : pos + 1;
    }
    return;
  }

  const int wm = wave_id >> 2, wn = wave_id & 3;
  const int lg = lane >> 4, lq = lane & 15;
  unsigned char* XT = smem;
  unsigned char* HT = smem + kXT;
  unsigned char* RING = smem + kXT + kHT;
  const int fr_row = lq * 128;
  const int fr_c0 = ((lg) ^ (lane & 7)) * 16;
  const int fr_c1 = ((lg + 4) ^ (lane & 7)) * 16;

  TFSTAMP(0)
  __syncthreads();
  TFSTAMP(1)
  {
    const int r = wave_id * 16 + (lane >> 2), q = lane & 3;
    uint4 raw[10];
    unsigned char* rowp = XT + r * 128;
#pragma unroll
    for (int i = 0; i < 10; ++i) {
      const int j = q + 4 * i;
      raw[i] = *(const uint4*)(rowp + (j >> 3) * (kBM * 128) + (((j & 7) ^ (r & 7)) << 4));
    }
    float f[10][8];
    float sm = 0.f;
#pragma unroll
    for (int i = 0; i < 10; ++i) {
      Chunk<bf16_t>::unpack(raw[i], f[i]);
#pragma unroll
      for (int e = 0; e < 8; ++e) sm += f[i][e];
    }
    sm += dpp_f<0xB1>(sm);
    sm += dpp_f<0x4E>(sm);
    const float mean = sm * (1.0f / kC);
    float qq = 0.f;
#pragma unroll
    for (int i = 0; i < 10; ++i)
#pragma unroll
      for (int e = 0; e < 8; ++e) { const float d = f[i][e] - mean; qq += d * d; }
    qq += dpp_f<0xB1>(qq);
    qq += dpp_f<0x4E>(qq);
    const float rstd = 1.0f / sqrtf(qq * (1.0f / kC) + p.eps);
#pragma unroll
    for (int i = 0; i < 10; ++i) {
      const int j = q + 4 * i;
      float y[8];
#pragma unroll
      for (int e = 0; e < 8; ++e) y[e] = (f[i][e] - mean) * rstd;
      *(uint4*)(rowp + (j >> 3) * (kBM * 128) + (((j & 7) ^ (r & 7)) << 4)) = Chunk<bf16_t>::pack(y);
    }
  }
  TFSTAMP(2)
  __syncthreads();
  TFSTAMP(3)

  f32x4 acc2[5][4];
#pragma unroll
  for (int a = 0; a < 5; ++a)
#pragma unroll
    for (int b = 0; b < 4; ++b) acc2[a][b] = f32x4{0.f, 0.f, 0.f, 0.f};

  unsigned uoff = 0;
  const unsigned char* xrow = XT + (wm * 64) * 128 + fr_row;
  const unsigned char* hrow = HT + (wm * 64) * 128 + fr_row;
  constexpr unsigned RM = (unsigned)(kRing - 1);
  int c = start;
  for (int ci = 0; ci < p.nchunks; ++ci, c = (c + 1 == p.nchunks) ? 0 : c + 1) {
    f32x4 acc1[2][4];
#pragma unroll
    for (int a = 0; a < 2; ++a)
#pragma unroll
      for (int b = 0; b < 4; ++b) acc1[a][b] = f32x4{0.f, 0.f, 0.f, 0.f};
    if (ci == 5) { TFSTAMP(11) }
    const float* bp = p.bias1 + c * 128 + wn * 32 + lg * 4;
    const f32x4 bv = *(const f32x4*)bp, bg = *(const f32x4*)(bp + 16);
    auto gemm1_tile = [&](int kt, unsigned tile_off) __attribute__((always_inline)) {
      const unsigned char* w0 = RING + ((uoff + tile_off + (unsigned)(wn * 32) * 128u) & RM) + fr_row;
      const unsigned char* w1 = RING + ((uoff + tile_off + (unsigned)(wn * 32 + 16) * 128u) & RM) + fr_row;
      const unsigned char* xs = xrow + kt * (kBM * 128);
#pragma unroll
      for (int kg = 0; kg < 2; ++kg) {
        const int co = kg ? fr_c1 : fr_c0;
        uint4 xf[4], wf[2];
        wf[0] = *(const uint4*)(w0 + co);
#pragma unroll
        for (int b = 0; b < 4; ++b) xf[b] = *(const uint4*)(xs + b * 2048 + co);
        wf[1] = *(const uint4*)(w1 + co);
#pragma unroll
        for (int a = 0; a < 2; ++a)
#pragma unroll
          for (int b = 0; b < 4; ++b) mma_kgroup<bf16_t>(wf[a], xf[b], acc1[a][b]);
      }
    };
    gemm1_tile(0, 0u);
    gemm1_tile(1, (unsigned)kW1Tile);
    __syncthreads();
    uoff = (uoff + 2u * kW1Tile) & RM;
    gemm1_tile(2, 0u);
    gemm1_tile(3, (unsigned)kW1Tile);
    __syncthreads();
    uoff = (uoff + 2u * kW1Tile) & RM;
    gemm1_tile(4, 0u);
#pragma unroll
    for (int b = 0; b < 4; ++b) {
      const f32x4 av = acc1[0][b] + bv, gv = acc1[1][b] + bg;
      const f32x4 o = TFDBG(p, 2) ? av * gv : av * gelu_erf_bf16_f4(gv);
      const int row = wm * 64 + b * 16 + lq;
      const int ch = wn * 2 + (lg >> 1);
      *(uint2*)(HT + row * 128 + ((ch ^ (row & 7)) << 4) + (lg & 1) * 8) = make_uint2(pack_bf16x2(o[0], o[1]), pack_bf16x2(o[2], o[3]));
    }
    __syncthreads();
    uoff = (uoff + (unsigned)kW1Tile) & RM;
    if (ci == 5) { TFSTAMP(12) }
#pragma unroll
    for (int kg = 0; kg < 2; ++kg) {
      const int co = kg ? fr_c1 : fr_c0;
      uint4 hf[4], wf[3];
#pragma unroll
      for (int b = 0; b < 4; ++b) hf[b] = *(const uint4*)(hrow + b * 2048 + co);
#pragma unroll
      for (int a = 0; a < 3; ++a) wf[a] = *(const uint4*)(RING + ((uoff + (unsigned)(wn * 48 + a * 16) * 128u) & RM) + fr_row + co);
#pragma unroll
      for (int a = 0; a < 3; ++a)
#pragma unroll
        for (int b = 0; b < 4; ++b) mma_kgroup<bf16_t>(wf[a], hf[b], acc2[a][b]);
    }
    __syncthreads();
    uoff = (uoff + (unsigned)kW2A) & RM;
#pragma unroll
    for (int kg = 0; kg < 2; ++kg) {
      const int co = kg ? fr_c1 : fr_c0;
      uint4 hf[4], wf[2];
#pragma unroll
      for (int b = 0; b < 4; ++b) hf[b] = *(const uint4*)(hrow + b * 2048 + co);
#pragma unroll
      for (int a = 0; a < 2; ++a) wf[a] = *(const uint4*)(RING + ((uoff + (unsigned)(wn * 32 + a * 16) * 128u) & RM) + fr_row + co);
#pragma unroll
      for (int a = 0; a < 2; ++a)
#pragma unroll
        for (int b = 0; b < 4; ++b) mma_kgroup<bf16_t>(wf[a], hf[b], acc2[3 + a][b]);
    }
    __syncthreads();
    uoff = (uoff + (unsigned)kW2B) & RM;
    if (ci == 0) { TFSTAMP(4) }
    if (ci == 5) { TFSTAMP(13) }
    if (ci == 9) { TFSTAMP(5) }
  }
  TFSTAMP(6)

  const int nl = wn * 80 + lg * 4;
  if constexpr (!PROJ) {
    constexpr int SROW = 80 * 4 + 16, CPR = 10, NCH = 160, NI = 3;
    unsigned char* stg = XT + wave_id * (16 * SROW);
    f32x4 b2[5];
#pragma unroll
    for (int a = 0; a < 5; ++a) b2[a] = *(const f32x4*)(p.bias2 + nl + a * 16);
    const int m_wave = m0 + wm * 64;
    uint4 rcur[NI], rnext[NI];
    auto load_res = [&](int b, uint4 (&r)[NI]) __attribute__((always_inline)) {
#pragma unroll
      for (int i = 0; i < NI; ++i) {
        const int cidx = lane + i * 64;
        const int row = cidx / CPR, cc = cidx - row * CPR;
        const int m = m_wave + b * 16 + row;
        if (cidx < NCH && m < p.M) r[i] = *(const uint4*)(p.x + (size_t)m * kC + wn * 80 + cc * 8);
      }
    };
    load_res(0, rcur);
#pragma unroll
    for (int b = 0; b < 4; ++b) {
#pragma unroll
      for (int a = 0; a < 5; ++a) *(f32x4*)(stg + lq * SROW + (a * 16 + lg * 4) * 4) = acc2[a][b] + b2[a];
      if (b + 1 < 4) load_res(b + 1, rnext);
      asm volatile("s_waitcnt lgkmcnt(0)" ::: "memory");
#pragma unroll
      for (int i = 0; i < NI; ++i) {
        const int cidx = lane + i * 64;
        if (cidx < NCH) {
          const int row = cidx / CPR, cc = cidx - row * CPR;
          const int m = m_wave + b * 16 + row;
          if (m < p.M) {
            float v[8], r[8];
            const unsigned char* sp = stg + row * SROW + cc * 32;
            const f32x4 t0 = *(const f32x4*)sp, t1 = *(const f32x4*)(sp + 16);
            Chunk<bf16_t>::unpack(rcur[i], r);
#pragma unroll
            for (int e = 0; e < 4; ++e) { v[e] = t0[e] + r[e]; v[4 + e] = t1[e] + r[4 + e]; }
            *(uint4*)(p.out + (size_t)m * kC + wn * 80 + cc * 8) = Chunk<bf16_t>::pack(v);
          }
        }
      }
      asm volatile("s_waitcnt lgkmcnt(0)" ::: "memory");
#pragma unroll
      for (int i = 0; i < NI; ++i) rcur[i] = rnext[i];
    }
  } else {
    int zero;
    asm volatile("v_mov_b32 %0, 0" : "=v"(zero));
    const int elane = lane + zero;
    const int elg = elane >> 4, elq = elane & 15;
    const int efr_row = elq * 128;
    const int efr_c0 = ((elg) ^ (elane & 7)) * 16, efr_c1 = ((elg + 4) ^ (elane & 7)) * 16;
    const int enl = wn * 80 + elg * 4;
#pragma unroll
    for (int a = 0; a < 5; ++a) {
      const int n = enl + a * 16;
      const f32x4 b2 = *(const f32x4*)(p.bias2 + n);
      const int kt = n >> 6, ch = (n & 63) >> 3, half = (n >> 2) & 1;
#pragma unroll
      for (int b = 0; b < 4; ++b) {
        const int row = wm * 64 + b * 16 + elq;
        const int m = m0 + row;
        uint2 rr = make_uint2(0u, 0u);
        if (m < p.M) rr = *(const uint2*)(p.x + (size_t)m * kC + n);
        f32x4 v = acc2[a][b] + b2;
        v[0] += bits_f32(rr.x << 16); v[1] += bits_f32(rr.x & 0xffff0000u);
        v[2] += bits_f32(rr.y << 16); v[3] += bits_f32(rr.y & 0xffff0000u);
        *(uint2*)(XT + kt * (kBM * 128) + row * 128 + ((ch ^ (row & 7)) << 4) + half * 8) =
            make_uint2(pack_bf16x2(v[0], v[1]), pack_bf16x2(v[2], v[3]));
      }
    }
    TFSTAMP(7)
    __syncthreads();
    TFSTAMP(8)
    const int pm = wave_id >> 1, pn = wave_id & 1;
    f32x4 acc3[2][5][2];
#pragma unroll
    for (int h = 0; h < 2; ++h)
#pragma unroll
      for (int a = 0; a < 5; ++a)
#pragma unroll
        for (int b = 0; b < 2; ++b) acc3[h][a][b] = f32x4{0.f, 0.f, 0.f, 0.f};
    const unsigned char* prow = XT + (pm * 32) * 128 + efr_row;
#pragma unroll 1
    for (int kt = 0; kt < kKT; ++kt) {
      const unsigned char* xs = prow + kt * (kBM * 128);
#pragma unroll
      for (int h = 0; h < 2; ++h) {
#pragma unroll
        for (int kg = 0; kg < 2; ++kg) {
          const int co = kg ? efr_c1 : efr_c0;
          uint4 xf[2], wf[5];
#pragma unroll
          for (int b = 0; b < 2; ++b) xf[b] = *(const uint4*)(xs + b * 2048 + co);
#pragma unroll
          for (int a = 0; a < 5; ++a)
            wf[a] = *(const uint4*)(RING + ((uoff + (unsigned)(pn * 80 + a * 16) * 128u) & (unsigned)(kRing - 1)) + efr_row + co);
#pragma unroll
          for (int a = 0; a < 5; ++a)
#pragma unroll
            for (int b = 0; b < 2; ++b) mma_kgroup<bf16_t>(wf[a], xf[b], acc3[h][a][b]);
        }
        __syncthreads();
        uoff = (uoff + kPUnit) & (unsigned)(kRing - 1);
      }
    }
    TFSTAMP(9)
    constexpr int SROW = 80 * 4 + 16, CPR = 10, NCH = 160, NI = 3;
    unsigned char* stg = HT + wave_id * (16 * SROW);
    uint4 rcur[NI], rnext[NI];
    auto load_res = [&](int blk, uint4 (&r)[NI]) __attribute__((always_inline)) {
#pragma unroll
      for (int i = 0; i < NI; ++i) {
        const int cidx = elane + i * 64;
        const int row = cidx / CPR, cc = cidx - row * CPR;
        const int m = m0 + pm * 32 + (blk & 1) * 16 + row;
        if (cidx < NCH && m < p.M) r[i] = *(const uint4*)(p.x2 + (size_t)m * kC + (blk >> 1) * 160 + pn * 80 + cc * 8);
      }
    };
    load_res(0, rcur);
#pragma unroll
    for (int h = 0; h < 2; ++h) {
      f32x4 b3[5];
#pragma unroll
      for (int a = 0; a < 5; ++a) b3[a] = *(const f32x4*)(p.bias3 + h * 160 + pn * 80 + a * 16 + elg * 4);
#pragma unroll
      for (int b = 0; b < 2; ++b) {
        const int blk = h * 2 + b;
#pragma unroll
        for (int a = 0; a < 5; ++a) *(f32x4*)(stg + elq * SROW + (a * 16 + elg * 4) * 4) = acc3[h][a][b] + b3[a];
        if (blk + 1 < 4) load_res(blk + 1, rnext);
        asm volatile("s_waitcnt lgkmcnt(0)" ::: "memory");
#pragma unroll
        for (int i = 0; i < NI; ++i) {
          const int cidx = elane + i * 64;
          if (cidx < NCH) {
            const int row = cidx / CPR, cc = cidx - row * CPR;
            const int m = m0 + pm * 32 + b * 16 + row;
            if (m < p.M) {
              float v[8], r[8];
              const unsigned char* sp = stg + row * SROW + cc * 32;
              const f32x4 t0 = *(const f32x4*)sp, t1 = *(const f32x4*)(sp + 16);
              Chunk<bf16_t>::unpack(rcur[i], r);
#pragma unroll
              for (int e = 0; e < 4; ++e) { v[e] = t0[e] + r[e]; v[4 + e] = t1[e] + r[4 + e]; }
              *(uint4*)(p.out + (size_t)m * kC + h * 160 + pn * 80 + cc * 8) = Chunk<bf16_t>::pack(v);
            }
          }
        }
        asm volatile("s_waitcnt lgkmcnt(0)" ::: "memory");
#pragma unroll
        for (int i = 0; i < NI; ++i) rcur[i] = rnext[i];
      }
    }
  }
  TFSTAMP(10)
}

__global__ __launch_bounds__(256) void tf_pack_stream_kernel(const bf16_t* __restrict__ w1, const bf16_t* __restrict__ w2,
                                                             const bf16_t* __restrict__ wp, uint4* __restrict__ out,
                                                             int nchunks, long long nvec) {
  const long long gid = (long long)blockIdx.x * 256 + threadIdx.x;
  if (gid >= nvec) return;
  const long long byte = gid * 16;
  const long long chunk_end = (long long)nchunks * kChunkBytes;
  const bf16_t* src;
  if (byte < chunk_end) {
    const int c = (int)(byte / kChunkBytes);
    const int o = (int)(byte - (long long)c * kChunkBytes);
    if (o < kKT * kW1Tile) {
      const int kt = o / kW1Tile, rem = o - kt * kW1Tile;
      const int r = rem >> 7, pc = (rem & 127) >> 4, lc = pc ^ (r & 7);
      src = w1 + (size_t)(c * 128 + r) * kC + kt * 64 + lc * 8;
    } else {
      const int rem = o - kKT * kW1Tile;
      const int r = rem >> 7, pc = (rem & 127) >> 4, lc = pc ^ (r & 7);
      const int n = r < 192 ? (r / 48) * 80 + (r % 48) : ((r - 192) / 32) * 80 + 48 + ((r - 192) % 32);
      src = w2 + (size_t)n * (4 * kC) + c * kHC + lc * 8;
    }
  } else {
    const int o = (int)(byte - chunk_end);
    const int kt = o / (2 * kPUnit), rem = o - kt * (2 * kPUnit);
    const int h = rem / kPUnit, rem2 = rem - h * kPUnit;
    const int r = rem2 >> 7, pc = (rem2 & 127) >> 4, lc = pc ^ (r & 7);
    if (r >= kC / 2) { out[gid] = make_uint4(0u, 0u, 0u, 0u); return; }
    src = wp + (size_t)(h * 160 + r) * kC + kt * 64 + lc * 8;
  }
  out[gid] = *(const uint4*)src;
}

int g_tfuse_dbg = 0;
int g_tfuse_mode = 3;

}

bool mlp_fused_ok(int C, int dtype) { return (g_tfuse_mode & 1) && C == kC && dtype == DT_BF16; }
bool mlp_fused_proj() { return (g_tfuse_mode & 2) != 0; }
void mlp_fused_set_mode(int m) { g_tfuse_mode = m & 3; }
void mlp_fused_set_dbg(int f) { g_tfuse_dbg = f; }
int mlp_fused_get_mode() { return g_tfuse_mode; }
size_t mlp_fused_stream_bytes(int C) { return C == kC ? (size_t)(4 * kC / kHC) * kChunkBytes + (size_t)2 * kKT * kPUnit : 0; }

int launch_pack_mlp_stream(const void* w1, const void* w2, const void* wp, void* out, int C, hipStream_t s) {
  if (C != kC || !w1 || !w2 || !wp || !out) return -2;
  const long long nvec = (long long)mlp_fused_stream_bytes(C) / 16;
  hipLaunchKernelGGL(tf_pack_stream_kernel, dim3((unsigned)((nvec + 255) / 256)), dim3(256), 0, s, (const bf16_t*)w1,
                     (const bf16_t*)w2, (const bf16_t*)wp, (uint4*)out, 4 * kC / kHC, nvec);
  return hipGetLastError() == hipSuccess ? 0 : -3;
}

int launch_mlp_fused(const void* h, void* out, const void* x2, const void* stream, const float* bias1, const float* bias2,
                     const float* bias3, const void* zeros, int M, int C, float eps, int proj, int rows_per_image, hipStream_t s) {
  if (C != kC || M < 1 || !h || !out || !stream || !bias1 || !bias2 || !zeros || (proj && (!x2 || !bias3))) return -2;
  MlpFusedParams p;
  p.x = (const bf16_t*)h; p.out = (bf16_t*)out; p.x2 = (const bf16_t*)x2;
  p.stream = (const unsigned char*)stream; p.bias1 = bias1; p.bias2 = bias2; p.bias3 = bias3; p.zeros = zeros;
  p.M = M; p.nchunks = 4 * kC / kHC; p.eps = eps;
  p.dbg = g_tfuse_dbg & 0xff;
  p.ldr_delay = (g_tfuse_dbg >> 16) & 3;
  p.rot_tiles = (!(g_tfuse_dbg & 256) && rows_per_image > 0 && rows_per_image % kBM == 0) ? rows_per_image / kBM : 0;
  const dim3 grid((M + kBM - 1) / kBM), block(768);
  static bool attr_set[64] = {};
  int dev = 0;
  if (hipGetDevice(&dev) != hipSuccess || dev < 0 || dev >= 64) dev = 0;
  if (!attr_set[dev]) {
    (void)hipFuncSetAttribute((const void*)mlp_fused_kernel<false>, hipFuncAttributeMaxDynamicSharedMemorySize, kLds);
    (void)hipFuncSetAttribute((const void*)mlp_fused_kernel<true>, hipFuncAttributeMaxDynamicSharedMemorySize, kLds);
    attr_set[dev] = true;
  }
  if (proj) LDMSEG_LAUNCH_GEMM("mlp_fused<bf16,proj=1>", mlp_fused_kernel<true>, grid, block, kLds, s, p);
  else LDMSEG_LAUNCH_GEMM("mlp_fused<bf16,proj=0>", mlp_fused_kernel<false>, grid, block, kLds, s, p);
  return hipGetLastError() == hipSuccess ? 0 : -3;
}

}

#ifdef LDMSEG_TFUSE_ABLATE
extern "C" int ldmseg_debug_tf_stamps(unsigned long long* host, int n) {
  return hipMemcpyFromSymbol(host, HIP_SYMBOL(ldmseg::g_tf_ts), (size_t)n * sizeof(unsigned long long)) == hipSuccess ? 0 : -1;
}
#endif
```

### latent-diffusion-segmentation_amd/csrc/tproj.hip

```cpp
#include <hip/hip_runtime.h>

#include "common.h"
#include "kernels.h"

namespace ldmseg {
namespace {

constexpr int kBM = 128, kC = 320, kKT = kC / 64;
constexpr int kXT = kKT * kBM * 128;
constexpr int kRing = 2 * 40960;
constexpr int kLds = kXT + kRing;
__device__ __forceinline__ unsigned ring_wrap(unsigned u) { return u >= (unsigned)kRing ? u - (unsigned)kRing : u; }
constexpr int kUnit = kC * 128;
constexpr int kNPass = 4;
constexpr int kUnitsPerPass = kKT;
constexpr int kStreamBytes = kNPass * kUnitsPerPass * kUnit;

__device__ __forceinline__ void glds16(const void* gsrc, unsigned lds_dst) {
  asm volatile(
      "s_mov_b32 m0, %1\n\t"
      "s_nop 0\n\t"
      "global_load_lds_dwordx4 %0, off"
      :
      : "v"(gsrc), "s"(lds_dst)
      : "memory");
}
__device__ __forceinline__ void glds16x2_sbase(unsigned voff, const void* sbase, unsigned lds_dst) {
  asm volatile(
      "s_mov_b32 m0, %2\n\t"
      "s_nop 3\n\t"
      "global_load_lds_dwordx4 %0, %1\n\t"
      "global_load_lds_dwordx4 %0, %1 offset:1024"
      :
      : "v"(voff), "s"(sbase), "s"(lds_dst)
      : "memory");
}
__device__ __forceinline__ void wait_pieces(int n) {
  switch (n) {
#define TP_W(N) case N: asm volatile("s_waitcnt vmcnt(" #N ")" ::: "memory"); break;
    TP_W(0) TP_W(1) TP_W(2) TP_W(3) TP_W(4) TP_W(5) TP_W(6) TP_W(7) TP_W(8) TP_W(9) TP_W(10) TP_W(11) TP_W(12) TP_W(13)
    TP_W(14) TP_W(15)
#undef TP_W
    default: asm volatile("s_waitcnt vmcnt(16)" ::: "memory"); break;
  }
}

#ifdef LDMSEG_TPROJ_ABLATE
#define TPDBG(bit) ((LDMSEG_TPROJ_ABLATE) & (bit))
#else
#define TPDBG(bit) 0
#endif

__device__ __forceinline__ void lds_barrier() { asm volatile("s_waitcnt lgkmcnt(0)\n\ts_barrier" ::: "memory"); }

struct ProjQkvParams {
  const bf16_t* x;
  bf16_t* h;
  bf16_t* qkv;
  const unsigned char* stream;
  const float* bias;
  const void* zeros;
  int M;
  float eps;
  int rot, stagger;
  const float* gn_partial;
  const float* gn_gamma;
  const float* gn_beta;
  int gn_nchunk, gn_per, gn_hw;
  float gn_eps;
};
constexpr int kCPG = kC / 32;
constexpr int kGnMaxChunks = 64;

__global__ __launch_bounds__(768, 3) void proj_ln_qkv_kernel(const ProjQkvParams p) {
  extern __shared__ __attribute__((aligned(16))) unsigned char smem[];
  const int tid = threadIdx.x, lane = tid & 63;
  const int wave_id = __builtin_amdgcn_readfirstlane(tid >> 6);
  const int m0 = blockIdx.x * kBM;
  const unsigned lds0 = (unsigned)(uintptr_t)((__attribute__((address_space(3))) unsigned char*)smem);
  constexpr int nunits = kNPass * kUnitsPerPass;
  if ((p.rot & 2) && ((blockIdx.x >> 3) & 1)) {
    for (int i = 0; i < p.stagger; ++i) __builtin_amdgcn_s_sleep(127);
  }

  if (wave_id >= 8) {
    const int lw = wave_id - 8;
    {
      const int ld_r = lane >> 3, ld_j = (lane & 7) ^ ld_r;
#pragma unroll 4
      for (int i = 0; i < (kKT * kBM / 8) / 4; ++i) {
        const int q = lw + 4 * i;
        const int kt = q >> 4, rg = q & 15;
        const int m = m0 + rg * 8 + ld_r;
        const void* src = m < p.M ? (const void*)((const unsigned char*)p.x + (size_t)m * (kC * 2) + kt * 128 + ld_j * 16) : p.zeros;
        glds16(src, __builtin_amdgcn_readfirstlane(lds0 + kt * (kBM * 128) + rg * 1024));
      }
    }
    __builtin_amdgcn_s_setprio(3);
    int left = nunits * 10;
    int iss = 0;
    const unsigned voff = (unsigned)lane * 16u;
    const int blk = (lw + ((p.rot & 1) ? (int)(blockIdx.x >> 3) : 0)) & 3;
    const unsigned char* src = p.stream + (size_t)blk * 2048;
    unsigned dst = (unsigned)blk * 2048u;
    auto issue_n = [&](int n) __attribute__((always_inline)) {
      for (int i = 0; i < n && left > 0; i += 2) {
        const unsigned long long su = (unsigned long long)(uintptr_t)src;
        const unsigned lo = __builtin_amdgcn_readfirstlane((unsigned)su), hi = __builtin_amdgcn_readfirstlane((unsigned)(su >> 32));
        if (!TPDBG(1)) glds16x2_sbase(voff, (const void*)(uintptr_t)(((unsigned long long)hi << 32) | lo), __builtin_amdgcn_readfirstlane(lds0 + (unsigned)kXT + dst));
        src += 8192;
        dst = ring_wrap(dst + 8192u);
        iss += 2;
        left -= 2;
      }
    };
    issue_n(20);
    int land = 10;
    wait_pieces(iss - land);
    __syncthreads();
    if (p.gn_partial) asm volatile("s_barrier" ::: "memory");
    for (int t = 0; t < nunits; ++t) {
      if (t == kUnitsPerPass) {
        asm volatile("s_barrier" ::: "memory");
        asm volatile("s_barrier" ::: "memory");
      }
      if (t + 1 < nunits) {
        land += 10;
        wait_pieces(iss - land);
      }
      asm volatile("s_barrier" ::: "memory");
      issue_n(10);
    }
    return;
  }

  const int lg = lane >> 4, lq = lane & 15;
  unsigned char* XT = smem;
  unsigned char* RING = smem + kXT;
  const int fr_row = lq * 128;
  const int fr_c0 = ((lg) ^ (lane & 7)) * 16;
  const int fr_c1 = ((lg + 4) ^ (lane & 7)) * 16;
  const int wm = wave_id >> 2, wn = wave_id & 3;
  const unsigned char* prow = XT + (wm * 64) * 128 + fr_row;
  unsigned uoff = 0;

  f32x4 bnext[5];
#pragma unroll
  for (int a = 0; a < 5; ++a) bnext[a] = *(const f32x4*)(p.bias + wn * 80 + a * 16 + lg * 4);
  float ga[8], gb[8];
  const int gn_j = tid % 40, gn_rg = tid / 40;
  if (p.gn_partial) {
    const int img = m0 / p.gn_hw;
    const int g = lane >> 1, half = lane & 1;
    const float2* src = (const float2*)p.gn_partial + (size_t)img * p.gn_nchunk * 32 + g;
    float2 e[kGnMaxChunks / 2];
    float cnt[kGnMaxChunks / 2];
#pragma unroll
    for (int i = 0; i < kGnMaxChunks / 2; ++i) {
      const int ch = half + 2 * i;
      const int p0 = ch * p.gn_per, np = min(p.gn_hw, p0 + p.gn_per) - p0;
      const bool ok = ch < p.gn_nchunk && np > 0;
      e[i] = src[(size_t)(ok ? ch : 0) * 32];
      cnt[i] = ok ? (float)(np * kCPG) : 0.f;
    }
    const float K = __shfl(e[0].x, lane & ~1);
    float n = 0.f, sd = 0.f;
#pragma unroll
    for (int i = 0; i < kGnMaxChunks / 2; ++i) { n += cnt[i]; sd += cnt[i] * (e[i].x - K); }
    auto pair_sum = [&](float v) __attribute__((always_inline)) {
      const float w = __shfl_xor(v, 1);
      return half ? w + v : v + w;
    };
    n = pair_sum(n);
    sd = pair_sum(sd);
    const float dbar = n > 0.f ? sd / n : 0.f;
    float m2 = 0.f;
#pragma unroll
    for (int i = 0; i < kGnMaxChunks / 2; ++i) {
      const float d = (e[i].x - K) - dbar;
      m2 += cnt[i] > 0.f ? e[i].y + cnt[i] * d * d : 0.f;
    }
    m2 = pair_sum(m2);
    const float g_mean = K + dbar;
    const float g_rstd = 1.0f / sqrtf((n > 0.f ? m2 / n : 0.f) + p.gn_eps);
    const int c0 = gn_j * 8;
    const int g0 = c0 / kCPG, g1 = min(g0 + 1, 31);
    const int split = min(8, (g0 + 1) * kCPG - c0);
    const float m_lo = __shfl(g_mean, 2 * g0), r_lo = __shfl(g_rstd, 2 * g0);
    const float m_hi = __shfl(g_mean, 2 * g1), r_hi = __shfl(g_rstd, 2 * g1);
    const f32x4 gm0 = *(const f32x4*)(p.gn_gamma + c0), gm1 = *(const f32x4*)(p.gn_gamma + c0 + 4);
    const f32x4 bt0 = *(const f32x4*)(p.gn_beta + c0), bt1 = *(const f32x4*)(p.gn_beta + c0 + 4);
#pragma unroll
    for (int e = 0; e < 8; ++e) {
      const float gam = e < 4 ? gm0[e & 3] : gm1[e & 3], bet = e < 4 ? bt0[e & 3] : bt1[e & 3];
      ga[e] = (e < split ? r_lo : r_hi) * gam;
      gb[e] = bet - (e < split ? m_lo : m_hi) * ga[e];
    }
  }
  lds_barrier();
  if (p.gn_partial) {
    if (gn_rg < 12) {
      unsigned char* colp = XT + (gn_j >> 3) * (kBM * 128);
#pragma unroll 2
      for (int row = gn_rg; row < kBM; row += 12) {
        unsigned char* q = colp + row * 128 + (((gn_j & 7) ^ (row & 7)) << 4);
        float f[8];
        Chunk<bf16_t>::unpack(*(const uint4*)q, f);
#pragma unroll
        for (int e = 0; e < 8; ++e) f[e] = f[e] * ga[e] + gb[e];
        *(uint4*)q = Chunk<bf16_t>::pack(f);
      }
    }
    lds_barrier();
  }

#pragma unroll 1
  for (int pass = 0; pass < kNPass; ++pass) {
    f32x4 acc[5][4];
#pragma unroll
    for (int a = 0; a < 5; ++a)
#pragma unroll
      for (int b = 0; b < 4; ++b) acc[a][b] = bnext[a];
#pragma unroll 1
    for (int kt = 0; kt < kKT; ++kt) {
      const unsigned char* xs = prow + kt * (kBM * 128);
      const unsigned char* ws = RING + uoff + (wn * 80) * 128 + fr_row;
#pragma unroll
      for (int kg = 0; kg < 2; ++kg) {
        const int co = kg ? fr_c1 : fr_c0;
        uint4 xf[4], wf[5];
        if (TPDBG(8)) {
#pragma unroll
          for (int b = 0; b < 4; ++b) xf[b] = make_uint4(lane, kt, kg, b);
#pragma unroll
          for (int a = 0; a < 5; ++a) wf[a] = make_uint4(lane, kt, kg, a);
        } else {
#pragma unroll
          for (int b = 0; b < 4; ++b) xf[b] = *(const uint4*)(xs + b * 2048 + co);
#pragma unroll
          for (int a = 0; a < 5; ++a) wf[a] = *(const uint4*)(ws + a * 2048 + co);
        }
        if (TPDBG(4)) {
#pragma unroll
          for (int a = 0; a < 5; ++a)
#pragma unroll
            for (int b = 0; b < 4; ++b) acc[a][b][0] += bits_f32(wf[a].x ^ xf[b].y);
        } else {
#pragma unroll
          for (int a = 0; a < 5; ++a)
#pragma unroll
            for (int b = 0; b < 4; ++b) mma_kgroup<bf16_t>(wf[a], xf[b], acc[a][b]);
        }
      }
      lds_barrier();
      uoff = uoff ? 0u : (unsigned)kUnit;
    }
    bf16_t* obase = pass == 0 ? p.h : p.qkv + (pass - 1) * kC;
    const int ldo = pass == 0 ? kC : 3 * kC;
    int zero;
    asm volatile("v_mov_b32 %0, 0" : "=v"(zero));
    const int elq = lq + zero, elg = lg + zero;
    const int n0 = wn * 80;
    if (pass + 1 < kNPass) {
#pragma unroll
      for (int a = 0; a < 5; ++a) bnext[a] = *(const f32x4*)(p.bias + (pass + 1) * kC + n0 + a * 16 + elg * 4);
    }
#pragma unroll
    for (int b = 0; b < 4; ++b) {
      const int row = wm * 64 + b * 16 + elq;
      uint2 pk[5];
#pragma unroll
      for (int a = 0; a < 5; ++a) {
        const f32x4 v = acc[a][b];
        pk[a] = make_uint2(pack_bf16x2(v[0], v[1]), pack_bf16x2(v[2], v[3]));
      }
      if (pass == 0) {
#pragma unroll
        for (int a = 0; a < 5; ++a) {
          const int n = n0 + a * 16 + elg * 4;
          const int kt = n >> 6, ch = (n & 63) >> 3, half = (n >> 2) & 1;
          *(uint2*)(XT + kt * (kBM * 128) + row * 128 + ((ch ^ (row & 7)) << 4) + half * 8) = pk[a];
        }
      }
      bf16_t* orow = obase + (size_t)(m0 + row) * ldo + n0;
#pragma unroll
      for (int a = 0; a < 4; a += 2) {
        const auto sx = __builtin_amdgcn_permlane16_swap(pk[a].x, pk[a + 1].x, false, false);
        const auto sy = __builtin_amdgcn_permlane16_swap(pk[a].y, pk[a + 1].y, false, false);
        if (!TPDBG(2)) *(uint4*)(orow + (a + (elg & 1)) * 16 + (elg >> 1) * 8) = make_uint4(sx[0], sy[0], sx[1], sy[1]);
      }
      if (!TPDBG(2)) *(uint2*)(orow + 4 * 16 + elg * 4) = pk[4];
    }
    if (pass == 0) {
      lds_barrier();
      const int r = wave_id * 16 + (lane >> 2), q = lane & 3;
      uint4 raw[10];
      unsigned char* rowp = XT + r * 128;
#pragma unroll
      for (int i = 0; i < 10; ++i) {
        const int j = q + 4 * i;
        raw[i] = *(const uint4*)(rowp + (j >> 3) * (kBM * 128) + (((j & 7) ^ (r & 7)) << 4));
      }
      float sm = 0.f;
#pragma unroll
      for (int i = 0; i < 10; ++i) {
        float f[8];
        Chunk<bf16_t>::unpack(raw[i], f);
#pragma unroll
        for (int e = 0; e < 8; ++e) sm += f[e];
      }
      sm += dpp_f<0xB1>(sm);
      sm += dpp_f<0x4E>(sm);
      const float mean = sm * (1.0f / kC);
      float qq = 0.f;
#pragma unroll
      for (int i = 0; i < 10; ++i) asm volatile("" : "+v"(raw[i].x), "+v"(raw[i].y), "+v"(raw[i].z), "+v"(raw[i].w));
#pragma unroll
      for (int i = 0; i < 10; ++i) {
        float f[8];
        Chunk<bf16_t>::unpack(raw[i], f);
#pragma unroll
        for (int e = 0; e < 8; ++e) { const float d = f[e] - mean; qq += d * d; }
      }
      qq += dpp_f<0xB1>(qq);
      qq += dpp_f<0x4E>(qq);
      const float rstd = 1.0f / sqrtf(qq * (1.0f / kC) + p.eps);
#pragma unroll
      for (int i = 0; i < 10; ++i) asm volatile("" : "+v"(raw[i].x), "+v"(raw[i].y), "+v"(raw[i].z), "+v"(raw[i].w));
#pragma unroll
      for (int i = 0; i < 10; ++i) {
        const int j = q + 4 * i;
        float f[8], y[8];
        Chunk<bf16_t>::unpack(raw[i], f);
#pragma unroll
        for (int e = 0; e < 8; ++e) y[e] = (f[e] - mean) * rstd;
        *(uint4*)(rowp + (j >> 3) * (kBM * 128) + (((j & 7) ^ (r & 7)) << 4)) = Chunk<bf16_t>::pack(y);
      }
      lds_barrier();
    }
  }
}

__global__ __launch_bounds__(256) void tp_pack_stream_kernel(const bf16_t* __restrict__ wp, const bf16_t* __restrict__ wqkv, uint4* __restrict__ out,
                                                             long long nvec) {
  const long long gid = (long long)blockIdx.x * 256 + threadIdx.x;
  if (gid >= nvec) return;
  const int byte = (int)(gid * 16);
  const int pass = byte / (kUnitsPerPass * kUnit), o = byte - pass * (kUnitsPerPass * kUnit);
  const int kt = o / kUnit, rem = o - kt * kUnit;
  const int r = rem >> 7, pc = (rem & 127) >> 4, lc = pc ^ (r & 7);
  const bf16_t* w = pass == 0 ? wp : wqkv + (size_t)(pass - 1) * kC * kC;
  out[gid] = *(const uint4*)(w + (size_t)r * kC + kt * 64 + lc * 8);
}

int g_tproj_mode = 3;

}

bool proj_qkv_fused_ok(int C, int M, int dtype) { return (g_tproj_mode & 1) && C == kC && dtype == DT_BF16 && M > 0 && M % kBM == 0; }
bool proj_qkv_gn_fold_ok(int HW) { return HW > 0 && HW % kBM == 0; }
int proj_qkv_gn_chunks(int B, int HW) {
  int n = 512 / (B > 0 ? B : 1);
  if (n > kGnMaxChunks) n = kGnMaxChunks;
  if (n < 4) n = 4;
  while (n > 1 && HW / n < 32) n >>= 1;
  return n;
}
void proj_qkv_set_mode(int m) { g_tproj_mode = m & 0xff; }
int proj_qkv_get_mode() { return g_tproj_mode; }
size_t proj_qkv_stream_bytes(int C) { return C == kC ? (size_t)kStreamBytes : 0; }

int launch_pack_proj_qkv_stream(const void* wp, const void* wqkv, void* out, int C, hipStream_t s) {
  if (C != kC || !wp || !wqkv || !out) return -2;
  const long long nvec = kStreamBytes / 16;
  hipLaunchKernelGGL(tp_pack_stream_kernel, dim3((unsigned)((nvec + 255) / 256)), dim3(256), 0, s, (const bf16_t*)wp, (const bf16_t*)wqkv, (uint4*)out, nvec);
  return hipGetLastError() == hipSuccess ? 0 : -3;
}

int launch_proj_qkv_fused(const void* x, void* h, void* qkv, const void* stream, const float* bias4, const void* zeros, int M, int C, float eps,
                          const GnFold* gn, hipStream_t s) {
  if (C != kC || M < 1 || M % kBM || !x || !h || !qkv || !stream || !bias4 || !zeros) return -2;
  ProjQkvParams p;
  p.x = (const bf16_t*)x; p.h = (bf16_t*)h; p.qkv = (bf16_t*)qkv; p.stream = (const unsigned char*)stream; p.bias = bias4; p.zeros = zeros;
  p.M = M; p.eps = eps; p.rot = (g_tproj_mode >> 1) & 3; p.stagger = (g_tproj_mode >> 4) & 15;
  p.gn_partial = nullptr; p.gn_gamma = p.gn_beta = nullptr; p.gn_nchunk = p.gn_per = p.gn_hw = 0; p.gn_eps = 0.f;
  if (gn) {
    if (!gn->partial || !gn->gamma || !gn->beta || !proj_qkv_gn_fold_ok(gn->HW) || M % gn->HW || gn->nchunk < 1 || gn->nchunk > kGnMaxChunks) return -2;
    p.gn_partial = gn->partial; p.gn_gamma = gn->gamma; p.gn_beta = gn->beta;
    p.gn_nchunk = gn->nchunk; p.gn_per = (gn->HW + gn->nchunk - 1) / gn->nchunk; p.gn_hw = gn->HW; p.gn_eps = gn->eps;
  }
  static bool attr_set[64] = {};
  int dev = 0;
  if (hipGetDevice(&dev) != hipSuccess || dev < 0 || dev >= 64) dev = 0;
  if (!attr_set[dev]) {
    (void)hipFuncSetAttribute((const void*)proj_ln_qkv_kernel, hipFuncAttributeMaxDynamicSharedMemorySize, kLds);
    attr_set[dev] = true;
  }
  LDMSEG_LAUNCH_GEMM(gn ? "proj_ln_qkv<bf16,gn>" : "proj_ln_qkv<bf16>", proj_ln_qkv_kernel, dim3(M / kBM), dim3(768), kLds, s, p);
  return hipGetLastError() == hipSuccess ? 0 : -3;
}

}
```

### latent-diffusion-segmentation_amd/ldmseg_amd/_lib.py

```python
import ctypes as C
import os

_HERE = os.path.dirname(os.path.abspath(__file__))
LIB_PATH = os.environ.get("LDMSEG_HIP_LIB") or os.path.join(_HERE, "libldmseg_hip.so")

F32, BF16, BF16X3 = 0, 1, 2
PRED = {"epsilon": 0, "sample": 1, "v_prediction": 2}


class UNetCfg(C.Structure):
    _fields_ = [("in_channels", C.c_int32), ("cross_attention", C.c_int32),
                ("compute_dtype", C.c_int32), ("device", C.c_int32)]


class VAECfg(C.Structure):
    _fields_ = [("in_channels", C.c_int32), ("int_channels", C.c_int32), ("out_channels", C.c_int32),
                ("latent_channels", C.c_int32), ("num_latents", C.c_int32), ("num_upscalers", C.c_int32),
                ("upscale_channels", C.c_int32), ("norm_num_groups", C.c_int32),
                ("block_out_channels", C.c_int32 * 4), ("compute_dtype", C.c_int32), ("device", C.c_int32)]


class VAEImageCfg(C.Structure):
    _fields_ = [("compute_dtype", C.c_int32), ("device", C.c_int32)]


class ClipVisionCfg(C.Structure):
    _fields_ = [("hidden_size", C.c_int32), ("intermediate_size", C.c_int32), ("num_layers", C.c_int32),
                ("num_heads", C.c_int32), ("image_size", C.c_int32), ("patch_size", C.c_int32),
                ("projection_dim", C.c_int32), ("compute_dtype", C.c_int32), ("device", C.c_int32)]


class ClipTextCfg(C.Structure):
    _fields_ = [("vocab_size", C.c_int32), ("max_positions", C.c_int32), ("hidden_size", C.c_int32),
                ("intermediate_size", C.c_int32), ("num_layers", C.c_int32), ("num_heads", C.c_int32),
                ("compute_dtype", C.c_int32), ("device", C.c_int32)]


class SampleCfg(C.Structure):
    _fields_ = [("n_steps", C.c_int32), ("timesteps", C.POINTER(C.c_int64)), ("coef", C.POINTER(C.c_float)),
                ("prediction_type", C.c_int32), ("clip_sample", C.c_int32), ("self_condition", C.c_int32),
                ("clip_sample_range", C.c_float),
                ("known_dev", C.c_void_p), ("z0_dev", C.c_void_p), ("noise_dev", C.c_void_p),
                ("paste_coef", C.POINTER(C.c_float))]


_vp, _i, _i64, _f, _sz, _d = C.c_void_p, C.c_int, C.c_int64, C.c_float, C.c_size_t, C.c_double

SIGNATURES = {
    "ldmseg_unet_create": (_i, [C.POINTER(UNetCfg), _i, C.POINTER(C.c_char_p), C.POINTER(_vp), C.POINTER(_i64), C.POINTER(_vp)]),
    "ldmseg_unet_destroy": (None, [_vp]),
    "ldmseg_unet_forward": (_i, [_vp, _vp, _vp, _i, _i64, _i, _i, _vp, _vp]),
    "ldmseg_unet_forward_parts": (_i, [_vp, _vp, _vp, _vp, _vp, _i, _i64, _i, _i, _vp, _vp]),
    "ldmseg_unet_forward_ctx": (_i, [_vp, _vp, _vp, _i, _i64, _i, _i, _vp, _i, _i, _vp, _vp]),
    "ldmseg_unet_workspace_bytes": (_sz, [_vp, _i, _i]),
    "ldmseg_unet_num_params": (_i64, [_vp]),
    "ldmseg_vae_create": (_i, [C.POINTER(VAECfg), _i, C.POINTER(C.c_char_p), C.POINTER(_vp), C.POINTER(_i64), C.POINTER(_vp)]),
    "ldmseg_vae_destroy": (None, [_vp]),
    "ldmseg_vae_decode": (_i, [_vp, _vp, _f, _i, _i, _i, _vp, _vp]),
    "ldmseg_vae_decode_argmax": (_i, [_vp, _vp, _f, _i, _i, _f, _i64, _vp, _vp, _vp]),
    "ldmseg_vae_encode": (_i, [_vp, _vp, _f, _f, _i, _i, _vp, _vp]),
    "ldmseg_vae_posterior": (_i, [_vp, _vp, _f, _i, _i, _vp, _vp]),
    "ldmseg_vae_num_params": (_i64, [_vp]),
    "ldmseg_ddim_step": (_i, [_vp, _vp, _f, _f, _f, _f, _i, _i, _f, _i, _vp, _vp, _sz, _vp]),
    "ldmseg_add_noise": (_i, [_vp, _vp, _vp, _vp, _i, _f, _vp, _i, _sz, _vp]),
    "ldmseg_remove_noise": (_i, [_vp, _vp, _vp, _vp, _i, _f, _vp, _i, _sz, _vp]),
    "ldmseg_unet_reserve": (_i, [_vp, _i, _i]),
    "ldmseg_unet_set_attention_fp8": (_i, [_vp, _i]),
    "ldmseg_unet_gn_fallbacks": (_i, [_vp, _vp]),
    "ldmseg_unet_gn_backoff": (_i, [_vp, _vp]),
    "ldmseg_unet_cf_fallbacks": (_i, [_vp, _vp]),
    "ldmseg_sample_loop": (_i, [_vp, C.POINTER(SampleCfg), _vp, _vp, _i, _i, _vp, _vp]),
    "ldmseg_sample_loop_guided": (_i, [_vp, C.POINTER(SampleCfg), _vp, _vp, _i, _i, _vp, _i, _i, _i, C.c_float, _vp, _vp]),
    "ldmseg_vae_image_create": (_i, [_vp, _i, _vp, _vp, _vp, _vp]),
    "ldmseg_vae_image_destroy": (None, [_vp]),
    "ldmseg_vae_image_num_params": (_i64, [_vp]),
    "ldmseg_vae_image_encode": (_i, [_vp, _vp, _f, _f, _i, _i, _i, _vp, _vp]),
    "ldmseg_clip_vision_create": (_i, [_vp, _i, _vp, _vp, _vp, _vp]),
    "ldmseg_clip_vision_destroy": (None, [_vp]),
    "ldmseg_clip_vision_num_params": (_i64, [_vp]),
    "ldmseg_clip_vision_forward": (_i, [_vp, _vp, _i, _vp, _vp, _vp]),
    "ldmseg_clip_vision_describe": (_i, [_vp, _vp, _i, _i, _i, C.POINTER(C.c_float), C.POINTER(C.c_float), _vp, _vp, _vp]),
    "ldmseg_clip_text_create": (_i, [_vp, _i, _vp, _vp, _vp, _vp]),
    "ldmseg_clip_text_destroy": (None, [_vp]),
    "ldmseg_clip_text_num_params": (_i64, [_vp]),
    "ldmseg_clip_text_forward": (_i, [_vp, _vp, _i, _i, _vp, _vp]),
    "ldmseg_vae_decode_panoptic": (_i, [_vp, _vp, _f, _i, _i, _i, _i, _vp, _vp, _vp, _i, _i, _f, _i, _d, _i64, _vp, _vp, _vp, _vp, _vp,
                                        _vp]),
    "ldmseg_semseg_meter_update": (_i, [_vp, _vp, _i64, _i, _i64, _vp, _vp]),
    "ldmseg_pq_match": (_i, [_vp, _vp, _i, _i, _vp, _vp, _vp, _vp, _i, _vp, _i] + [_vp] * 8),
    "ldmseg_vae_decode_semseg": (_i, [_vp, _vp, _f, _i, _i, _i, _i, _f, _i64, _vp, _i64, _i, _vp, _vp, _vp]),
    "ldmseg_vae_reconstruct_semseg": (_i, [_vp, _vp, _f, _f, _i, _i, _i, _i, _f, _i64, _vp, _i64, _i, _vp, _vp, _vp]),
    "ldmseg_vae_reconstruct_panoptic": (_i, [_vp, _vp, _f, _f, _i, _i, _i, _i, _vp, _vp, _vp, _i, _f, _i, _d, _i64, _vp, _vp, _vp, _vp,
                                             _vp, _vp]),
    "ldmseg_panoptic_postprocess": (_i, [_vp, _i, _i, _i, _i, _i, _i, _f, _i, _d, _i64, _vp, _vp, _vp, _vp, _vp, _vp]),
    "ldmseg_bit_encode": (_i, [_vp, _i, _i, _i, _i64, _f, _f, _f, _vp, _vp, _vp]),
    "ldmseg_bit_decode": (_i, [_vp, _i, _i, _i, _vp, _vp]),
    "ldmseg_last_error": (C.c_char_p, []),
    "ldmseg_version": (C.c_char_p, []),
    "ldmseg_profile_enable": (_i, [_i]),
    "ldmseg_profile_read": (_i, [_i, C.POINTER(_i64), C.POINTER(C.c_double), C.POINTER(C.c_double), C.POINTER(C.c_double)]),
    "ldmseg_profile_reset": (_i, []),
    "ldmseg_profile_dump": (_i, [C.c_char_p]),
    "ldmseg_debug_set": (_i, [_i, _i]),
    "ldmseg_debug_get": (_i, [_i]),
    "ldmseg_op_conv2d": (_i, [_vp, _vp, _vp, _vp, _i, _i, _i, _i, _i, _i, _i, _i, _i, _i, _vp, _vp]),
    "ldmseg_op_linear": (_i, [_vp, _vp, _vp, _vp, _vp, _i, _i, _i, _i, _i, _i, _i, _i, _vp, _vp]),
    "ldmseg_op_groupnorm": (_i, [_vp, _vp, _vp, _vp, _i, _i, _i, _i, _f, _i, _i, _vp, _vp]),
    "ldmseg_op_layernorm": (_i, [_vp, _vp, _vp, _i, _i, _f, _i, _i, _vp, _vp]),
    "ldmseg_op_attention": (_i, [_vp, _i, _i, _i, _i, _i, _vp, _vp]),
    "ldmseg_op_attention_causal": (_i, [_vp, _i, _i, _i, _i, _i, _vp, _vp]),
    "ldmseg_op_clip_text_tokens": (_i, [_vp, _vp, _vp, _i, _i, _i, _i, _i, _vp, _vp]),
    "ldmseg_op_clip_text_final_ln": (_i, [_vp, _vp, _vp, _i, _i, _f, _i, _vp, _vp]),
    "ldmseg_op_attention_cross": (_i, [_vp, _vp, _i, _i, _i, _i, _i, _i, _vp, _vp]),
    "ldmseg_op_attention_fp8": (_i, [_vp, _i, _i, _i, _i, _vp, _i, C.POINTER(C.c_float), _vp]),
    "ldmseg_op_convt2": (_i, [_vp, _vp, _vp, _i, _i, _i, _i, _i, _i, _vp, _vp]),
    "ldmseg_op_bilinear2x": (_i, [_vp, _i, _i, _i, _i, _i, _vp, _vp]),
    "ldmseg_op_chained_ff_out": (_i, [_vp, _vp, _vp, _vp, _vp, _vp, _vp, _i, _i, _i, _i, _vp, _vp]),
    "ldmseg_op_igemm": (_i, [_vp, _vp, _vp, _vp, _vp, _vp, _i, _i, _i, _i, _i, _i, _i, _i, _i, _i, _i, _i, _i, _vp, _vp]),
    "ldmseg_op_conv3x3_plus_1x1": (_i, [_vp, _vp, _vp, _vp, _vp, _vp, _vp, _i, _i, _i, _i, _i, _i, _i, _i, _i, _vp, _i, C.POINTER(C.c_float), _vp]),
    "ldmseg_op_ln_linear": (_i, [_vp, _vp, _vp, _vp, _vp, _i, _i, _i, _f, _i, _i, _vp, _vp]),
    "ldmseg_op_ln_linear_silu": (_i, [_vp, _vp, _vp, _vp, _vp, _i, _i, _i, _f, _i, _vp, _vp]),
    "ldmseg_op_clip_patch_rows": (_i, [_vp, _i, _i, _i, _i, _i, C.POINTER(C.c_float), C.POINTER(C.c_float), _i, _i, _vp, _vp]),
    "ldmseg_op_conv_out_tail": (_i, [_vp, _vp, _vp, _i, _i, _i, _vp, _i, _i, C.POINTER(C.c_float), _i, _i, _f, _vp, _vp, _vp, _vp, _vp,
                                     _vp, _f, _f, _vp, _vp]),
    "ldmseg_op_transformer_ff": (_i, [_vp] * 10 + [_i, _i, _f, _i, _i, _vp, _i, C.POINTER(C.c_float), _vp]),
    "ldmseg_op_transformer_in": (_i, [_vp] * 8 + [_i, _i, _f, _i, _i, _vp, _vp, _i, C.POINTER(C.c_float), _vp]),
    "ldmseg_op_gn_transformer_in": (_i, [_vp] * 3 + [_f, _i, _i] + [_vp] * 7 + [_i, _i, _f, _i, _i, _vp, _vp, _i, C.POINTER(C.c_float), _vp]),
    "ldmseg_bench_igemm": (_i, [_vp, _vp, _vp, _vp, _vp, _vp, _i, _i, _i, _i, _i, _i, _i, _i, _i, _i, _i, _i, _i, _i,
                                C.POINTER(C.c_float), _vp]),
    "ldmseg_bench_attention": (_i, [_vp, _i, _i, _i, _i, _i, _i, C.POINTER(C.c_float), _vp]),
    "ldmseg_op_panoptic_from_decoder": (_i, [_vp, _i, _i, _i, _i, _i, _i, _i, _vp, _vp, _vp, _i, _i, _f, _i, _d, _i64, _vp, _vp, _vp,
                                             _vp, _vp, _vp, _vp]),
    "ldmseg_op_semseg_from_decoder": (_i, [_vp, _i, _i, _i, _i, _i, _i, _i, _f, _i64, _vp, _i64, _i, _vp, _vp, _vp, _vp]),
    "ldmseg_op_conv_groupnorm": (_i, [_vp, _vp, _vp, _vp, _vp, _vp, _i, _i, _i, _i, _i, _f, _i, _i, _i, _vp, _vp]),
    "ldmseg_bench_groupnorm": (_i, [_vp, _vp, _i, _i, _i, _i, _i, _i, _i, C.POINTER(C.c_float), _vp]),
    "ldmseg_igemm_last_kernel": (_i, [C.c_char_p, _i]),
    "ldmseg_op_igemm_plan": (_i, [C.POINTER(_i), _i, _i, C.c_char_p, _i]),
    "ldmseg_op_groupnorm_plan": (_i, [_i, _i, _i, _i, _i, _i, _i, _i, C.c_char_p, _i]),
    "ldmseg_op_conv_groupnorm_plan": (_i, [_i, _i, _i, _i, C.c_char_p, _i]),
    "ldmseg_op_attention_plan": (_i, [_i, _i, _i, _i, _i, _i, _i, C.c_char_p, _i]),
    "ldmseg_op_fastdiv": (_i, [_vp, _i, _i, _vp, _vp]),
    "ldmseg_igemm_log": (_i, [_i]),
    "ldmseg_igemm_log_read": (_i, [C.c_char_p, _i]),
}

_lib = None


def lib():
    global _lib
    if _lib is None:
        if not os.path.exists(LIB_PATH):
            raise RuntimeError(
                f"{LIB_PATH} not found: the HIP extension is required (no CPU fallback). "
                "Run `python __graft_entry__.py build` or `python -m ldmseg_amd.build`.")
        h = C.CDLL(LIB_PATH)
        for name, (res, args) in SIGNATURES.items():
            if os.environ.get("LDMSEG_HIP_LIB") and not hasattr(h, name):
                continue
            fn = getattr(h, name)
            fn.restype = res
            fn.argtypes = args
        _lib = h
    return _lib


def check(code, what=""):
    if code != 0:
        msg = lib().ldmseg_last_error()
        raise RuntimeError(f"libldmseg_hip: {what} failed with code {code}: {msg.decode() if msg else ''}")


def igemm_last_kernel():
    buf = C.create_string_buffer(128)
    lib().ldmseg_igemm_last_kernel(buf, 128)
    return buf.value.decode()


LOG_ALL = 2


def igemm_log(enable):
    lib().ldmseg_igemm_log(int(enable))


def igemm_log_read():
    buf = C.create_string_buffer(1 << 16)
    check(lib().ldmseg_igemm_log_read(buf, 1 << 16), "ldmseg_igemm_log_read")
    return {ln for ln in buf.value.decode().split("\n") if ln}


def stream_ptr(device=None):
    import torch
    return C.c_void_p(torch.cuda.current_stream(device).cuda_stream)


def ptr(t):
    return C.c_void_p(t.data_ptr()) if t is not None else C.c_void_p(0)


def require_cuda_f32(t, name):
    import torch
    if not isinstance(t, torch.Tensor) or not t.is_cuda:
        raise RuntimeError(f"{name} must be a tensor on the MI355X (got {type(t).__name__}"
                           f"{'' if not isinstance(t, torch.Tensor) else ' on ' + str(t.device)}): "
                           "the HIP path has no CPU fallback")
    if t.dtype != torch.float32:
        t = t.float()
    return t.contiguous()


def weight_arrays(state_dict, device):
    import torch
    keep = []
    names = []
    for k, v in state_dict.items():
        t = v.detach().to(device=device, dtype=torch.float32).contiguous()
        keep.append(t)
        names.append(k.encode())
    n = len(keep)
    c_names = (C.c_char_p * n)(*names)
    c_ptrs = (C.c_void_p * n)(*[t.data_ptr() for t in keep])
    c_numels = (C.c_int64 * n)(*[t.numel() for t in keep])
    return n, c_names, c_ptrs, c_numels, keep
```

Measured before the change: 994.1 image-steps/s.

## Finer-grained weight streaming in fused MLP and proj-QKV kernels

Splits the LDS ring consumption in the fused transformer MLP and proj/LN/QKV kernels into smaller per-tile steps (7 units per chunk instead of 5 in the MLP, half-unit k-group steps in the projection). Loader waves release and issue smaller shares after each finer barrier, so weight loads run further ahead of compute. The projection weight packing layout and swizzle change to match the half-unit tiles. This adds more barriers per chunk, which could raise sync overhead. It also adds timestamp instrumentation and a rows-per-image variant of the transformer_ff op.

```diff
diff --git a/include/ldmseg_hip_ops.h b/include/ldmseg_hip_ops.h
--- a/include/ldmseg_hip_ops.h
+++ b/include/ldmseg_hip_ops.h
@@ -66,6 +66,9 @@
 int ldmseg_op_transformer_ff(const float* h, const float* x, const float* gamma, const float* beta, const float* w1, const float* b1,
                              const float* w2, const float* b2, const float* wp, const float* bp, int M, int C, float eps, int dtype,
                              int mode, float* out, int time_iters, float* us_per_call, void* stream);
+int ldmseg_op_transformer_ff_rows(const float* h, const float* x, const float* gamma, const float* beta, const float* w1, const float* b1,
+                                  const float* w2, const float* b2, const float* wp, const float* bp, int M, int C, float eps, int dtype,
+                                  int mode, int rows_per_image, float* out, int time_iters, float* us_per_call, void* stream);
 int ldmseg_op_conv_out_tail(const float* x, const float* w, const float* bias, int B, int H, int W, float* eps_out, int ddim, int last,
                             const float* coef4, int pred_type, int clip, float clip_range, float* latents, float* cond,
                             const float* rgb, const uint8_t* known, const float* z0, const float* noise, float sa, float sb,
diff --git a/latent-diffusion-segmentation_amd/csrc/engine.hip b/latent-diffusion-segmentation_amd/csrc/engine.hip
--- a/latent-diffusion-segmentation_amd/csrc/engine.hip
+++ b/latent-diffusion-segmentation_amd/csrc/engine.hip
@@ -2474,6 +2474,7 @@
   if (key == 8 || key == 11) return groupnorm_knob(key);
   if (key == 9) return igemm_get_cm_mode();
   if (key == 12) return mlp_fused_get_mode();
+  if (key == 13) return mlp_fused_get_dbg();
   if (key == 14) return step_tail_get_mode();
   if (key == 16) return proj_qkv_get_mode();
   if (key == 15) return attention_mx_get_mode();
diff --git a/latent-diffusion-segmentation_amd/csrc/kernels.h b/latent-diffusion-segmentation_amd/csrc/kernels.h
--- a/latent-diffusion-segmentation_amd/csrc/kernels.h
+++ b/latent-diffusion-segmentation_amd/csrc/kernels.h
@@ -203,6 +203,7 @@
 int launch_mlp_fused(const void* h, void* out, const void* x2, const void* stream, const float* bias1, const float* bias2,
                      const float* bias3, const void* zeros, int M, int C, float eps, int proj, int rows_per_image, hipStream_t s);
 void mlp_fused_set_dbg(int flags);
+int mlp_fused_get_dbg();
 const void* igemm_zero_page();
 
 int launch_rowstats(const void* x, float* stats, int M, int C, float eps, int dtype, hipStream_t s);
diff --git a/latent-diffusion-segmentation_amd/csrc/ops_api.hip b/latent-diffusion-segmentation_amd/csrc/ops_api.hip
--- a/latent-diffusion-segmentation_amd/csrc/ops_api.hip
+++ b/latent-diffusion-segmentation_amd/csrc/ops_api.hip
@@ -699,12 +699,12 @@
   return 0;
 }
 
-int ldmseg_op_transformer_ff(const float* h, const float* x, const float* gamma, const float* beta, const float* w1, const float* b1,
-                             const float* w2, const float* b2, const float* wp, const float* bp, int M, int C, float eps, int dtype,
-                             int mode, float* out, int time_iters, float* us_per_call, void* stream) {
-  hipStream_t s = (hipStream_t)stream;
-  Temp t;
-  const int rows_per_image = (M % 4096 == 0) ? 4096 : 0;
+int ldmseg_op_transformer_ff_rows(const float* h, const float* x, const float* gamma, const float* beta, const float* w1, const float* b1,
+                                  const float* w2, const float* b2, const float* wp, const float* bp, int M, int C, float eps, int dtype,
+                                  int mode, int rows_per_image, float* out, int time_iters, float* us_per_call, void* stream) {
+  hipStream_t s = (hipStream_t)stream;
+  Temp t;
+  if (rows_per_image < 0 || (rows_per_image > 0 && M % rows_per_image)) return -2;
   if (C % bke(dtype) || (mode != 0 && (dtype != DT_BF16 || !mlp_fused_stream_bytes(C)))) return -2;
   const int N1 = 8 * C;
   void* hp = t.get((size_t)M * C * es(dtype));
@@ -762,6 +762,12 @@
   if (time_iters > 0 && us_per_call) *us_per_call = time_launches(s, 2, time_iters, [&](int) { (void)run(); });
   from_dev_dtype(op, out, (size_t)M * C, dtype, s);
   return 0;
+}
+int ldmseg_op_transformer_ff(const float* h, const float* x, const float* gamma, const float* beta, const float* w1, const float* b1,
+                             const float* w2, const float* b2, const float* wp, const float* bp, int M, int C, float eps, int dtype,
+                             int mode, float* out, int time_iters, float* us_per_call, void* stream) {
+  return ldmseg_op_transformer_ff_rows(h, x, gamma, beta, w1, b1, w2, b2, wp, bp, M, C, eps, dtype, mode, (M % 4096 == 0) ? 4096 : 0, out,
+                                       time_iters, us_per_call, stream);
 }
 
 static int transformer_in_impl(const float* x, const float* gn_gamma, const float* gn_beta, float gn_eps, int gn_images, int gn_mode,
diff --git a/latent-diffusion-segmentation_amd/csrc/tfuse.hip b/latent-diffusion-segmentation_amd/csrc/tfuse.hip
--- a/latent-diffusion-segmentation_amd/csrc/tfuse.hip
+++ b/latent-diffusion-segmentation_amd/csrc/tfuse.hip
@@ -75,16 +75,18 @@
 };
 #ifdef LDMSEG_TFUSE_ABLATE
 #define TFDBG(p, bit) ((LDMSEG_TFUSE_ABLATE) & (bit))
-__device__ unsigned long long g_tf_ts[64];
+__device__ unsigned long long g_tf_ts[128];
 #define TFSTAMP(slot) if (blockIdx.x == 0 && threadIdx.x == 0) g_tf_ts[slot] = wall_clock64();
 #define TFSTAMP_L(slot, cond) if ((cond) && blockIdx.x == 0 && threadIdx.x == 512) g_tf_ts[slot] = wall_clock64();
+#define TFSTAMP_C(slot, cond) if ((cond) && blockIdx.x == 0 && threadIdx.x == 0) g_tf_ts[slot] = wall_clock64();
 #else
 #define TFDBG(p, bit) 0
 #define TFSTAMP(slot)
 #define TFSTAMP_L(slot, cond)
+#define TFSTAMP_C(slot, cond)
 #endif
 
-template <bool PROJ>
+template <bool PROJ, bool AHEAD>
 __global__ __launch_bounds__(768, 3) void mlp_fused_kernel(const MlpFusedParams p) {
   extern __shared__ __attribute__((aligned(16))) unsigned char smem[];
   const int tid = threadIdx.x;
@@ -92,7 +94,9 @@
   const int wave_id = __builtin_amdgcn_readfirstlane(tid >> 6);
   const int m0 = blockIdx.x * kBM;
   const unsigned lds0 = (unsigned)(uintptr_t)((__attribute__((address_space(3))) unsigned char*)smem);
-  const int nunits = p.nchunks * 5 + (PROJ ? 2 * kKT : 0);
+  constexpr int kUPC = AHEAD ? 7 : 5;
+  constexpr unsigned kShares = AHEAD ? 0x4644444u : 0x46488u;
+  const int nunits = p.nchunks * kUPC + (PROJ ? 2 * kKT : 0);
   const int start = p.rot_tiles > 0 ? (int)(((unsigned)blockIdx.x % (unsigned)p.rot_tiles) * 7u % (unsigned)p.nchunks) : 0;
 
   if (wave_id >= 8) {
@@ -109,7 +113,7 @@
       }
     }
     __builtin_amdgcn_s_setprio(3);
-    const int nchunk_units = p.nchunks * 5;
+    const int nchunk_units = p.nchunks * kUPC;
     const int chunk_pieces = p.nchunks * 30;
     int left = chunk_pieces + (PROJ ? 2 * kKT * 6 : 0);
     int iss = 0;
@@ -138,22 +142,27 @@
     issue_n(16);
     wait_pieces(iss);
     __syncthreads();
-    int land = 8;
+    int land = (int)(kShares & 15u);
     wait_pieces(iss - land);
     __syncthreads();
     int pos = 0;
     for (int t = 0; t < nunits; ++t) {
       if (PROJ && t == nchunk_units) asm volatile("s_barrier" ::: "memory");
-      const int sh_t = (t < nchunk_units) ? ((0x46488 >> (4 * pos)) & 15) : 6;
+      const int sh_t = (t < nchunk_units) ? (int)((kShares >> (4 * pos)) & 15u) : 6;
+      [[maybe_unused]] const bool stamp = t >= 5 * kUPC && t < 6 * kUPC;
+      TFSTAMP_L(24 + 4 * pos, stamp)
       if (t + 1 < nunits) {
-        const int pn = pos == 4 ? 0 : pos + 1;
-        land += (t + 1 < nchunk_units) ? ((0x46488 >> (4 * pn)) & 15) : 6;
+        const int pn = pos == kUPC - 1 ? 0 : pos + 1;
+        land += (t + 1 < nchunk_units) ? (int)((kShares >> (4 * pn)) & 15u) : 6;
         wait_pieces(iss - land);
       }
+      TFSTAMP_L(25 + 4 * pos, stamp)
       asm volatile("s_barrier" ::: "memory");
+      TFSTAMP_L(26 + 4 * pos, stamp)
       if (p.ldr_delay == 1) __builtin_amdgcn_s_sleep(2);
       issue_n(sh_t);
-      pos = (pos == 4) ? 0 : pos + 1;
+      TFSTAMP_L(27 + 4 * pos, stamp)
+      pos = (pos == kUPC - 1) ? 0 : pos + 1;
     }
     return;
   }
@@ -249,14 +258,29 @@
           for (int b = 0; b < 4; ++b) mma_kgroup<bf16_t>(wf[a], xf[b], acc1[a][b]);
       }
     };
-    gemm1_tile(0, 0u);
-    gemm1_tile(1, (unsigned)kW1Tile);
-    __syncthreads();
-    uoff = (uoff + 2u * kW1Tile) & RM;
-    gemm1_tile(2, 0u);
-    gemm1_tile(3, (unsigned)kW1Tile);
-    __syncthreads();
-    uoff = (uoff + 2u * kW1Tile) & RM;
+    auto step_end = [&](int j, unsigned bytes) __attribute__((always_inline)) {
+      TFSTAMP_C(64 + 2 * j, ci == 5)
+      __syncthreads();
+      TFSTAMP_C(65 + 2 * j, ci == 5)
+      uoff = (uoff + bytes) & RM;
+    };
+    if constexpr (AHEAD) {
+      gemm1_tile(0, 0u);
+      step_end(0, (unsigned)kW1Tile);
+      gemm1_tile(1, 0u);
+      step_end(1, (unsigned)kW1Tile);
+      gemm1_tile(2, 0u);
+      step_end(2, (unsigned)kW1Tile);
+      gemm1_tile(3, 0u);
+      step_end(3, (unsigned)kW1Tile);
+    } else {
+      gemm1_tile(0, 0u);
+      gemm1_tile(1, (unsigned)kW1Tile);
+      step_end(0, 2u * kW1Tile);
+      gemm1_tile(2, 0u);
+      gemm1_tile(3, (unsigned)kW1Tile);
+      step_end(1, 2u * kW1Tile);
+    }
     gemm1_tile(4, 0u);
 #pragma unroll
     for (int b = 0; b < 4; ++b) {
@@ -266,8 +290,7 @@
       const int ch = wn * 2 + (lg >> 1);
       *(uint2*)(HT + row * 128 + ((ch ^ (row & 7)) << 4) + (lg & 1) * 8) = make_uint2(pack_bf16x2(o[0], o[1]), pack_bf16x2(o[2], o[3]));
     }
-    __syncthreads();
-    uoff = (uoff + (unsigned)kW1Tile) & RM;
+    step_end(kUPC - 3, (unsigned)kW1Tile);
     if (ci == 5) { TFSTAMP(12) }
 #pragma unroll
     for (int kg = 0; kg < 2; ++kg) {
@@ -282,8 +305,7 @@
 #pragma unroll
         for (int b = 0; b < 4; ++b) mma_kgroup<bf16_t>(wf[a], hf[b], acc2[a][b]);
     }
-    __syncthreads();
-    uoff = (uoff + (unsigned)kW2A) & RM;
+    step_end(kUPC - 2, (unsigned)kW2A);
 #pragma unroll
     for (int kg = 0; kg < 2; ++kg) {
       const int co = kg ? fr_c1 : fr_c0;
@@ -297,8 +319,7 @@
 #pragma unroll
         for (int b = 0; b < 4; ++b) mma_kgroup<bf16_t>(wf[a], hf[b], acc2[3 + a][b]);
     }
-    __syncthreads();
-    uoff = (uoff + (unsigned)kW2B) & RM;
+    step_end(kUPC - 1, (unsigned)kW2B);
     if (ci == 0) { TFSTAMP(4) }
     if (ci == 5) { TFSTAMP(13) }
     if (ci == 9) { TFSTAMP(5) }
@@ -497,6 +518,7 @@
 }
 
 int g_tfuse_dbg = 0;
+constexpr bool kAheadDefault = true;
 int g_tfuse_mode = 3;
 
 }
@@ -505,6 +527,7 @@
 bool mlp_fused_proj() { return (g_tfuse_mode & 2) != 0; }
 void mlp_fused_set_mode(int m) { g_tfuse_mode = m & 3; }
 void mlp_fused_set_dbg(int f) { g_tfuse_dbg = f; }
+int mlp_fused_get_dbg() { return g_tfuse_dbg; }
 int mlp_fused_get_mode() { return g_tfuse_mode; }
 size_t mlp_fused_stream_bytes(int C) { return C == kC ? (size_t)(4 * kC / kHC) * kChunkBytes + (size_t)2 * kKT * kPUnit : 0; }
 
@@ -531,12 +554,18 @@
   int dev = 0;
   if (hipGetDevice(&dev) != hipSuccess || dev < 0 || dev >= 64) dev = 0;
   if (!attr_set[dev]) {
-    (void)hipFuncSetAttribute((const void*)mlp_fused_kernel<false>, hipFuncAttributeMaxDynamicSharedMemorySize, kLds);
-    (void)hipFuncSetAttribute((const void*)mlp_fused_kernel<true>, hipFuncAttributeMaxDynamicSharedMemorySize, kLds);
+    (void)hipFuncSetAttribute((const void*)mlp_fused_kernel<false, false>, hipFuncAttributeMaxDynamicSharedMemorySize, kLds);
+    (void)hipFuncSetAttribute((const void*)mlp_fused_kernel<true, false>, hipFuncAttributeMaxDynamicSharedMemorySize, kLds);
+    (void)hipFuncSetAttribute((const void*)mlp_fused_kernel<false, true>, hipFuncAttributeMaxDynamicSharedMemorySize, kLds);
+    (void)hipFuncSetAttribute((const void*)mlp_fused_kernel<true, true>, hipFuncAttributeMaxDynamicSharedMemorySize, kLds);
     attr_set[dev] = true;
   }
-  if (proj) LDMSEG_LAUNCH_GEMM("mlp_fused<bf16,proj=1>", mlp_fused_kernel<true>, grid, block, kLds, s, p);
-  else LDMSEG_LAUNCH_GEMM("mlp_fused<bf16,proj=0>", mlp_fused_kernel<false>, grid, block, kLds, s, p);
+  const int proto = (g_tfuse_dbg >> 18) & 3;
+  const bool ahead = proto == 0 ? kAheadDefault : proto == 2;
+  void (*const kp)(const MlpFusedParams) = proj ? (ahead ? mlp_fused_kernel<true, true> : mlp_fused_kernel<true, false>)
+                                                   : (ahead ? mlp_fused_kernel<false, true> : mlp_fused_kernel<false, false>);
+  if (proj) LDMSEG_LAUNCH_GEMM("mlp_fused<bf16,proj=1>", kp, grid, block, kLds, s, p);
+  else LDMSEG_LAUNCH_GEMM("mlp_fused<bf16,proj=0>", kp, grid, block, kLds, s, p);
   return hipGetLastError() == hipSuccess ? 0 : -3;
 }
 
diff --git a/latent-diffusion-segmentation_amd/csrc/tproj.hip b/latent-diffusion-segmentation_amd/csrc/tproj.hip
--- a/latent-diffusion-segmentation_amd/csrc/tproj.hip
+++ b/latent-diffusion-segmentation_amd/csrc/tproj.hip
@@ -12,6 +12,7 @@
 constexpr int kLds = kXT + kRing;
 __device__ __forceinline__ unsigned ring_wrap(unsigned u) { return u >= (unsigned)kRing ? u - (unsigned)kRing : u; }
 constexpr int kUnit = kC * 128;
+constexpr int kSub = kC * 64;
 constexpr int kNPass = 4;
 constexpr int kUnitsPerPass = kKT;
 constexpr int kStreamBytes = kNPass * kUnitsPerPass * kUnit;
@@ -47,8 +48,13 @@
 
 #ifdef LDMSEG_TPROJ_ABLATE
 #define TPDBG(bit) ((LDMSEG_TPROJ_ABLATE) & (bit))
+__device__ unsigned long long g_tp_ts[128];
+#define TPSTAMP_L(slot, cond) if ((cond) && blockIdx.x == 0 && threadIdx.x == 512) g_tp_ts[slot] = wall_clock64();
+#define TPSTAMP_C(slot, cond) if ((cond) && blockIdx.x == 0 && threadIdx.x == 0) g_tp_ts[slot] = wall_clock64();
 #else
 #define TPDBG(bit) 0
+#define TPSTAMP_L(slot, cond)
+#define TPSTAMP_C(slot, cond)
 #endif
 
 __device__ __forceinline__ void lds_barrier() { asm volatile("s_waitcnt lgkmcnt(0)\n\ts_barrier" ::: "memory"); }
@@ -72,13 +78,15 @@
 constexpr int kCPG = kC / 32;
 constexpr int kGnMaxChunks = 64;
 
+template <bool AHEAD>
 __global__ __launch_bounds__(768, 3) void proj_ln_qkv_kernel(const ProjQkvParams p) {
   extern __shared__ __attribute__((aligned(16))) unsigned char smem[];
   const int tid = threadIdx.x, lane = tid & 63;
   const int wave_id = __builtin_amdgcn_readfirstlane(tid >> 6);
   const int m0 = blockIdx.x * kBM;
   const unsigned lds0 = (unsigned)(uintptr_t)((__attribute__((address_space(3))) unsigned char*)smem);
-  constexpr int nunits = kNPass * kUnitsPerPass;
+  constexpr int kSteps = AHEAD ? 2 * kUnitsPerPass : kUnitsPerPass;
+  constexpr int nunits = kNPass * kSteps;
   if ((p.rot & 2) && ((blockIdx.x >> 3) & 1)) {
     for (int i = 0; i < p.stagger; ++i) __builtin_amdgcn_s_sleep(127);
   }
@@ -97,7 +105,7 @@
       }
     }
     __builtin_amdgcn_s_setprio(3);
-    int left = nunits * 10;
+    int left = kNPass * kUnitsPerPass * 10;
     int iss = 0;
     const unsigned voff = (unsigned)lane * 16u;
     const int blk = (lw + ((p.rot & 1) ? (int)(blockIdx.x >> 3) : 0)) & 3;
@@ -114,22 +122,28 @@
         left -= 2;
       }
     };
+    auto share = [&](int u) __attribute__((always_inline)) { return AHEAD ? ((((u & 1) != 0) == (blk < 2)) ? 4 : 6) : 10; };
     issue_n(20);
-    int land = 10;
+    int land = share(0);
     wait_pieces(iss - land);
     __syncthreads();
     if (p.gn_partial) asm volatile("s_barrier" ::: "memory");
     for (int t = 0; t < nunits; ++t) {
-      if (t == kUnitsPerPass) {
+      if (t == kSteps) {
         asm volatile("s_barrier" ::: "memory");
         asm volatile("s_barrier" ::: "memory");
       }
+      [[maybe_unused]] const bool stamp = t >= 2 * kSteps && t < 3 * kSteps;
+      TPSTAMP_L(4 * (t - 2 * kSteps), stamp)
       if (t + 1 < nunits) {
-        land += 10;
+        land += share(t + 1);
         wait_pieces(iss - land);
       }
+      TPSTAMP_L(4 * (t - 2 * kSteps) + 1, stamp)
       asm volatile("s_barrier" ::: "memory");
-      issue_n(10);
+      TPSTAMP_L(4 * (t - 2 * kSteps) + 2, stamp)
+      issue_n(share(t));
+      TPSTAMP_L(4 * (t - 2 * kSteps) + 3, stamp)
     }
     return;
   }
@@ -140,6 +154,7 @@
   const int fr_row = lq * 128;
   const int fr_c0 = ((lg) ^ (lane & 7)) * 16;
   const int fr_c1 = ((lg + 4) ^ (lane & 7)) * 16;
+  const int wfr = lq * 64 + ((lg ^ ((4 - (lq >> 2)) & 3)) << 4);
   const int wm = wave_id >> 2, wn = wave_id & 3;
   const unsigned char* prow = XT + (wm * 64) * 128 + fr_row;
   unsigned uoff = 0;
@@ -224,10 +239,10 @@
 #pragma unroll 1
     for (int kt = 0; kt < kKT; ++kt) {
       const unsigned char* xs = prow + kt * (kBM * 128);
-      const unsigned char* ws = RING + uoff + (wn * 80) * 128 + fr_row;
 #pragma unroll
       for (int kg = 0; kg < 2; ++kg) {
         const int co = kg ? fr_c1 : fr_c0;
+        const unsigned char* ws = RING + uoff + (AHEAD ? 0 : kg * kSub) + (wn * 80) * 64 + wfr;
         uint4 xf[4], wf[5];
         if (TPDBG(8)) {
 #pragma unroll
@@ -238,7 +253,7 @@
 #pragma unroll
           for (int b = 0; b < 4; ++b) xf[b] = *(const uint4*)(xs + b * 2048 + co);
 #pragma unroll
-          for (int a = 0; a < 5; ++a) wf[a] = *(const uint4*)(ws + a * 2048 + co);
+          for (int a = 0; a < 5; ++a) wf[a] = *(const uint4*)(ws + a * 1024);
         }
         if (TPDBG(4)) {
 #pragma unroll
@@ -251,9 +266,19 @@
 #pragma unroll
             for (int b = 0; b < 4; ++b) mma_kgroup<bf16_t>(wf[a], xf[b], acc[a][b]);
         }
-      }
-      lds_barrier();
-      uoff = uoff ? 0u : (unsigned)kUnit;
+        if constexpr (AHEAD) {
+          TPSTAMP_C(64 + 2 * (2 * kt + kg), pass == 2)
+          lds_barrier();
+          TPSTAMP_C(65 + 2 * (2 * kt + kg), pass == 2)
+          uoff = ring_wrap(uoff + (unsigned)kSub);
+        }
+      }
+      if constexpr (!AHEAD) {
+        TPSTAMP_C(64 + 2 * kt, pass == 2)
+        lds_barrier();
+        TPSTAMP_C(65 + 2 * kt, pass == 2)
+        uoff = uoff ? 0u : (unsigned)kUnit;
+      }
     }
     bf16_t* obase = pass == 0 ? p.h : p.qkv + (pass - 1) * kC;
     const int ldo = pass == 0 ? kC : 3 * kC;
@@ -348,12 +373,15 @@
   const int byte = (int)(gid * 16);
   const int pass = byte / (kUnitsPerPass * kUnit), o = byte - pass * (kUnitsPerPass * kUnit);
   const int kt = o / kUnit, rem = o - kt * kUnit;
-  const int r = rem >> 7, pc = (rem & 127) >> 4, lc = pc ^ (r & 7);
+  const int kg = rem / kSub, rem2 = rem - kg * kSub;
+  const int r = rem2 >> 6, pc = (rem2 & 63) >> 4, lc = pc ^ ((4 - (r >> 2)) & 3);
   const bf16_t* w = pass == 0 ? wp : wqkv + (size_t)(pass - 1) * kC * kC;
-  out[gid] = *(const uint4*)(w + (size_t)r * kC + kt * 64 + lc * 8);
+  out[gid] = *(const uint4*)(w + (size_t)r * kC + kt * 64 + kg * 32 + lc * 8);
 }
 
 int g_tproj_mode = 3;
+int g_tproj_proto = 0;
+constexpr bool kAheadDefault = true;
 
 }
 
@@ -366,8 +394,8 @@
   while (n > 1 && HW / n < 32) n >>= 1;
   return n;
 }
-void proj_qkv_set_mode(int m) { g_tproj_mode = m & 0xff; }
-int proj_qkv_get_mode() { return g_tproj_mode; }
+void proj_qkv_set_mode(int m) { g_tproj_mode = m & 0xff; g_tproj_proto = (m >> 8) & 3; }
+int proj_qkv_get_mode() { return g_tproj_mode | (g_tproj_proto << 8); }
 size_t proj_qkv_stream_bytes(int C) { return C == kC ? (size_t)kStreamBytes : 0; }
 
 int launch_pack_proj_qkv_stream(const void* wp, const void* wqkv, void* out, int C, hipStream_t s) {
@@ -393,11 +421,20 @@
   int dev = 0;
   if (hipGetDevice(&dev) != hipSuccess || dev < 0 || dev >= 64) dev = 0;
   if (!attr_set[dev]) {
-    (void)hipFuncSetAttribute((const void*)proj_ln_qkv_kernel, hipFuncAttributeMaxDynamicSharedMemorySize, kLds);
+    (void)hipFuncSetAttribute((const void*)proj_ln_qkv_kernel<false>, hipFuncAttributeMaxDynamicSharedMemorySize, kLds);
+    (void)hipFuncSetAttribute((const void*)proj_ln_qkv_kernel<true>, hipFuncAttributeMaxDynamicSharedMemorySize, kLds);
     attr_set[dev] = true;
   }
-  LDMSEG_LAUNCH_GEMM(gn ? "proj_ln_qkv<bf16,gn>" : "proj_ln_qkv<bf16>", proj_ln_qkv_kernel, dim3(M / kBM), dim3(768), kLds, s, p);
+  const bool ahead = g_tproj_proto == 0 ? kAheadDefault : g_tproj_proto == 2;
+  void (*const kp)(const ProjQkvParams) = ahead ? proj_ln_qkv_kernel<true> : proj_ln_qkv_kernel<false>;
+  LDMSEG_LAUNCH_GEMM(gn ? "proj_ln_qkv<bf16,gn>" : "proj_ln_qkv<bf16>", kp, dim3(M / kBM), dim3(768), kLds, s, p);
   return hipGetLastError() == hipSuccess ? 0 : -3;
 }
 
 }
+
+#ifdef LDMSEG_TPROJ_ABLATE
+extern "C" int ldmseg_debug_tp_stamps(unsigned long long* host, int n) {
+  return hipMemcpyFromSymbol(host, HIP_SYMBOL(ldmseg::g_tp_ts), (size_t)n * sizeof(unsigned long long)) == hipSuccess ? 0 : -1;
+}
+#endif
diff --git a/latent-diffusion-segmentation_amd/ldmseg_amd/_lib.py b/latent-diffusion-segmentation_amd/ldmseg_amd/_lib.py
--- a/latent-diffusion-segmentation_amd/ldmseg_amd/_lib.py
+++ b/latent-diffusion-segmentation_amd/ldmseg_amd/_lib.py
@@ -124,6 +124,7 @@
     "ldmseg_op_conv_out_tail": (_i, [_vp, _vp, _vp, _i, _i, _i, _vp, _i, _i, C.POINTER(C.c_float), _i, _i, _f, _vp, _vp, _vp, _vp, _vp,
                                      _vp, _f, _f, _vp, _vp]),
     "ldmseg_op_transformer_ff": (_i, [_vp] * 10 + [_i, _i, _f, _i, _i, _vp, _i, C.POINTER(C.c_float), _vp]),
+    "ldmseg_op_transformer_ff_rows": (_i, [_vp] * 10 + [_i, _i, _f, _i, _i, _i, _vp, _i, C.POINTER(C.c_float), _vp]),
     "ldmseg_op_transformer_in": (_i, [_vp] * 8 + [_i, _i, _f, _i, _i, _vp, _vp, _i, C.POINTER(C.c_float), _vp]),
     "ldmseg_op_gn_transformer_in": (_i, [_vp] * 3 + [_f, _i, _i] + [_vp] * 7 + [_i, _i, _f, _i, _i, _vp, _vp, _i, C.POINTER(C.c_float), _vp]),
     "ldmseg_bench_igemm": (_i, [_vp, _vp, _vp, _vp, _vp, _vp, _i, _i, _i, _i, _i, _i, _i, _i, _i, _i, _i, _i, _i, _i,
```

Result: no change. 993.9 image-steps/s (-0.0%).
